# aidilayce/FollowMyHold

Hardware: AMD Instinct MI355X
Metric: guidance-steps/sec (512x512, 778+20k verts) (higher is better)
Workload: dtype f32; 1 GPU; configs[1]: 512x512 frame/GPU, 778-vert hand + 10242-vert/20480-face object, joint step (phase C); images_per_gpu=1, global_images=1, parallelism=image-sharded x1, steps_per_graph=1

## Files before the change

### followmyhold_amd/csrc/foho_step.hip

```cpp
#include <hip/hip_runtime.h>
#include <hip/hip_fp16.h>
#include <stdint.h>
#include <stdlib.h>
#include <string.h>

#include <algorithm>
#include <string>

#include "../../include/foho_hip.h"
#include "foho_common.h"

using namespace foho;

static thread_local char g_err[256] = "";
void foho_set_error(const char* msg) {
    strncpy(g_err, msg, sizeof(g_err) - 1);
    g_err[sizeof(g_err) - 1] = 0;
}
extern "C" const char* foho_last_error(void) { return g_err; }
extern "C" int foho_version(void) { return 105; }
extern "C" int foho_abi_sizes(int64_t out[5]) {
    out[0] = sizeof(foho_image), out[1] = sizeof(foho_dims), out[2] = sizeof(foho_render_cfg), out[3] = sizeof(foho_step_cfg),
    out[4] = sizeof(foho_step_desc);
    return 105;
}

struct ProfState {
    hipEvent_t ev[32];
    const char* name[32];
    int n;
};
static thread_local ProfState* g_prof = nullptr;

#define CHECK_LAUNCH(kname_)                                                                   \
    do {                                                                                     \
        hipError_t e_ = hipGetLastError();                                                   \
        if (e_ != hipSuccess) {                                                              \
            char b_[200];                                                                    \
            snprintf(b_, sizeof(b_), "%s: %s", kname_, hipGetErrorString(e_));                 \
            foho_set_error(b_);                                                              \
            return FOHO_ERR_LAUNCH;                                                          \
        }                                                                                    \
        if (g_prof && g_prof->n < 32) {                                                      \
            g_prof->name[g_prof->n] = kname_;                                                  \
            (void)hipEventRecord(g_prof->ev[g_prof->n++], stream);                           \
        }                                                                                    \
    } while (0)

#include "foho_stamps.h"

constexpr int BTX = 32, BTY = 8;
constexpr int RF = 64;
constexpr int RQ_CAP = 1024;
constexpr int FRAC_SEG = 256;
constexpr int K_SIL = 100;
constexpr int KFIX_MAX = 32;
constexpr int KFIX_FRAGS = 1024;
constexpr int LOSS_BLOCKS = 256;
constexpr int NPART = 12;
constexpr int LOSS_SLOTS = 16;
constexpr int VERT_BLOCKS_MAX = 1024;
constexpr int SIM_NP = 20;
constexpr int VB = 64;
constexpr int VP_CAP = 1024;
constexpr int SIM_ROWS_MAX = VERT_BLOCKS_MAX * (256 / VB);
constexpr int NSTAT = 32;
constexpr int SIM_ACC = 40;
constexpr int STATE_NEXT = 64;
constexpr int PIX_BWD_TILE_BLOCKS = 256;
constexpr int BWD_SPLIT = 4;
constexpr int BWD_SLOTS = 512;

struct MeshInfo {
    unsigned long long kmin_inv[3];
    unsigned long long kmax[3];
};

struct FracEntry {
    int pix;
    int face;
    float sdist;
};
struct KFixEntry {
    int pix;
    int pad;
    unsigned long long thr;
};

constexpr int NSLOT = 64;
struct RSlot {
    unsigned hit_count;
    unsigned rgb_min_inv, rgb_max;
    unsigned disp_min_inv, disp_max;
    unsigned pad[11];
};
struct RStats {
    unsigned flags;
    unsigned pad[3];
};

struct WS {
    size_t total;
    size_t world, ndc, vn_raw, vn, mesh_info, face_ndc;
    size_t p2f, zbuf, sdist, prod, pcol, hit_list, hit_count, bwd_list, bwd_count, tile_touched, tile_clean, pair_v, pending, state_next, sim_acc;
    size_t zkey, fullb, nfrac, plog;
    size_t kfix_count, kfix;
    size_t clean_begin, clean_end;
    size_t frac, frac_count, frac_seg, seg_count, rstats, rslot, loss_part, stats2;
    int nseg;
    size_t g_ndc, g_nrm, g_world, g_direct;
    size_t knn_idx, knn_d2, kp3d, g_kp3d, vert_part, sim_part, xf_part, g_special, parity, int_count, final_ticket, knn_inv, loss_acc, vbox, hand_order;
    size_t tile_static, image_static, act_list, act_count;
    int btiles_x, nbtiles;
    size_t zero_begin, zero_end;
};

static inline size_t al(size_t x) { return (x + 255) & ~(size_t)255; }
static inline int cdiv(int a, int b) { return (a + b - 1) / b; }
static inline int vert_block(const foho_dims& d) { return d.B > 1 ? 2 * VB : VB; }
static inline int raster_faces_per_block(int F, int B = 1) {
    int r = 8;
    while (r < RF && (size_t)r * 256 < (size_t)F * B) r <<= 1;
    return r;
}
constexpr int RF_H_MIN = 2;
static inline void raster_blocks(const foho_dims& d, int& rf_h, int& rf_o, int& nRh, int& nRo, int hand_faces = 0) {
    const int Fh_max = d.Fh_max > 0 ? d.Fh_max : d.Fmax, Fo_max = d.Fo_max > 0 ? d.Fo_max : d.Fmax;
    rf_h = std::max(2, raster_faces_per_block(Fh_max, d.B) / 2);
    if (hand_faces > 0) rf_h = std::max(RF_H_MIN, std::min(hand_faces, RF));
    rf_o = raster_faces_per_block(Fo_max, d.B);
    if (const char* e = FOHO_DEV_ENV("FOHO_DEBUG_RFH")) rf_h = std::max(1, std::min(atoi(e), RF));
    if (const char* e = FOHO_DEV_ENV("FOHO_DEBUG_RFO")) rf_o = std::max(1, std::min(atoi(e), RF));
    nRh = cdiv(Fh_max, rf_h);
    nRo = cdiv(Fo_max, rf_o);
}

static WS make_ws(const foho_dims& d) {
    WS w;
    size_t o = 0;
    const size_t P = (size_t)d.H * d.W, R = d.n_renders, B = d.B;
    const size_t V3 = (size_t)d.Vtot * 3 * 4;
    w.btiles_x = (d.W + BTX - 1) / BTX;
    w.nbtiles = w.btiles_x * ((d.H + BTY - 1) / BTY);
    auto take = [&](size_t bytes) {
        size_t r = o;
        o = al(o + bytes);
        return r;
    };
    const int G1 = d.grid_res + 1;
    w.tile_static = take(B * (size_t)w.nbtiles * 12 * 4);
    w.image_static = take(B * 12 * 8);
    w.zero_begin = o;
    w.frac_count = take(R * B * 4);
    {
        int rf_h, rf_o, nRh, nRo;
#ifdef FOHO_NSEG_AUTO
        raster_blocks(d, rf_h, rf_o, nRh, nRo, 0);
#else
        raster_blocks(d, rf_h, rf_o, nRh, nRo, RF_H_MIN);
#endif
        w.nseg = nRh + nRo;
    }
    w.seg_count = take(R * B * (size_t)w.nseg * 4);
    w.kfix_count = take(R * B * 4);
    w.hit_count = take(R * B * 4);
    w.bwd_count = take(R * B * 4);
    w.rstats = take(R * B * sizeof(RStats));
    w.rslot = take(R * B * NSLOT * sizeof(RSlot));
    w.g_world = take(V3);
    w.g_ndc = take(V3);
    w.g_nrm = take(V3);
    w.parity = take(B * 2 * (size_t)G1 * G1 * 16);
    w.int_count = take(B * 4);
    w.final_ticket = take(B * 4);
    w.loss_acc = take(R * B * LOSS_SLOTS * NPART * 8);
    w.knn_inv = take(B * (size_t)std::max(d.Vh_max, 1) * 8);
    w.zero_end = o;
    w.clean_begin = o;
    w.zkey = take(R * B * P * 8);
    w.fullb = take(R * B * P);
    w.nfrac = take(R * B * P * 4);
    w.plog = take(R * B * P * 8);
    w.tile_touched = take(R * B * (size_t)w.nbtiles);
    w.tile_clean = take(R * B * (size_t)w.nbtiles);
    w.sim_acc = take(2 * B * (size_t)SIM_ACC * 4);
    w.pending = take(B * 4);
    w.clean_end = o;
    w.mesh_info = take(B * 2 * sizeof(MeshInfo));
    w.xf_part = take(B * 2 * VERT_BLOCKS_MAX * 8 * 4);
    w.vbox = take(B * (size_t)VERT_BLOCKS_MAX * 4 * 8 * 4);
    w.world = take(V3);
    w.ndc = take(V3);
    w.vn_raw = take((size_t)d.Vtot * 16);
    w.vn = take(V3);
    w.face_ndc = take((size_t)d.Ftot * 9 * 4);
    w.state_next = take(B * (size_t)STATE_NEXT * 4);
    w.pair_v = take((size_t)d.Ftot * 3 * 8);
    w.p2f = take(R * B * P * 4);
    w.zbuf = take(R * B * P * 4);
    w.sdist = take(R * B * P * 4);
    w.prod = take(R * B * P * 4);
    w.hit_list = take(R * B * (size_t)w.nbtiles * 4);
    w.bwd_list = take(R * B * (size_t)w.nbtiles * BWD_SPLIT * 4);
    w.pcol = take(R * B * P * 12);
    w.frac = take(R * B * (size_t)d.frac_cap * sizeof(FracEntry));
    w.frac_seg = take(R * B * (size_t)w.nseg * FRAC_SEG * sizeof(FracEntry));
    w.act_list = take(R * B * (size_t)w.nbtiles * 4);
    w.act_count = take(R * B * 4);
    w.kfix = take(R * B * KFIX_MAX * sizeof(KFixEntry));
    w.loss_part = take(R * B * LOSS_BLOCKS * NPART * 4);
    w.stats2 = take(R * B * NSTAT * 4);
    w.g_direct = take(V3);
    w.knn_idx = take((size_t)d.Vtot * 4);
    w.knn_d2 = take((size_t)d.Vtot * 4);
    w.hand_order = take(B * (size_t)std::max(d.Vh_max, 1) * 4);
    w.kp3d = take(B * 21 * 3 * 4);
    w.g_kp3d = take(B * 21 * 3 * 4);
    w.vert_part = take(B * VERT_BLOCKS_MAX * 8 * 4);
    w.g_special = take(B * 2 * 6 * 4 * 4);
    w.sim_part = take(B * 2 * (size_t)SIM_ROWS_MAX * SIM_NP * 4);
    w.total = o;
    return w;
}

extern "C" size_t foho_step_workspace_bytes(const foho_dims* dims) {
    if (!dims) return 0;
    return make_ws(*dims).total;
}

extern "C" int64_t foho_step_workspace_region(const foho_dims* dims, int region, int64_t* nbytes) {
    if (!dims) return -1;
    const WS w = make_ws(*dims);
    const foho_dims& d = *dims;
    const size_t P = (size_t)d.H * d.W, R = d.n_renders, B = d.B, V3 = (size_t)d.Vtot * 12;
    const int G1 = d.grid_res + 1;
    size_t off, n;
    switch (region) {
        case FOHO_WS_WORLD: off = w.world; n = V3; break;
        case FOHO_WS_NDC: off = w.ndc; n = V3; break;
        case FOHO_WS_VN: off = w.vn; n = V3; break;
        case FOHO_WS_P2F: off = w.p2f; n = R * B * P * 4; break;
        case FOHO_WS_ZBUF: off = w.zbuf; n = R * B * P * 4; break;
        case FOHO_WS_SDIST: off = w.sdist; n = R * B * P * 4; break;
        case FOHO_WS_PROD: off = w.prod; n = R * B * P * 4; break;
        case FOHO_WS_KNN_IDX: off = w.knn_idx; n = (size_t)d.Vtot * 4; break;
        case FOHO_WS_KNN_D2: off = w.knn_d2; n = (size_t)d.Vtot * 4; break;
        case FOHO_WS_GWORLD: off = w.g_world; n = V3; break;
        case FOHO_WS_FRAC_COUNT: off = w.frac_count; n = R * B * 4; break;
        case FOHO_WS_STATS: off = w.stats2; n = R * B * NSTAT * 4; break;
        case FOHO_WS_PARITY: off = w.parity; n = B * 2 * (size_t)G1 * G1 * 16; break;
        case FOHO_WS_FRAG_COUNT: off = w.nfrac; n = R * B * P * 4; break;
        case FOHO_WS_SEG_COUNT: off = w.seg_count; n = R * B * (size_t)w.nseg * 4; break;
        case FOHO_WS_HAND_ORDER: off = w.hand_order; n = B * (size_t)std::max(d.Vh_max, 1) * 4; break;
        default: return -1;
    }
    if (nbytes) *nbytes = (int64_t)n;
    return (int64_t)off;
}

__device__ __forceinline__ unsigned long long pack_pair(int v0, int v1, int v2, int corner) {
    return (unsigned long long)((unsigned)v0 & 0x3FFFFFu) | ((unsigned long long)((unsigned)(v1 - v0 + (1 << 19)) & 0xFFFFFu) << 22) |
           ((unsigned long long)((unsigned)(v2 - v0 + (1 << 19)) & 0xFFFFFu) << 42) | ((unsigned long long)(corner & 3) << 62);
}
__device__ __forceinline__ void unpack_pair(unsigned long long p, int v[3], int& corner) {
    v[0] = (int)(p & 0x3FFFFFu);
    v[1] = v[0] + (int)((p >> 22) & 0xFFFFFu) - (1 << 19);
    v[2] = v[0] + (int)((p >> 42) & 0xFFFFFu) - (1 << 19);
    corner = (int)(p >> 62);
}

struct Ctx {
    foho_dims d;
    PixAxis ax, ay;
    const foho_image* img;
    const float* verts_in;
    const int32_t* faces;
    const int32_t *inc_off, *inc_fc, *nbr_off, *nbr_idx;
    const float* J;
    const float *tgt_normal, *tgt_disp;
    const uint8_t* mask;
    const float* kps_2d;
    float *params, *adam_m, *adam_v;
    int32_t* adam_t;
    float *losses, *grad_params, *grad_verts_in;
    int32_t* flags;
    float *world, *ndc, *vn_raw, *vn;
    MeshInfo* mesh_info;
    float* face_ndc;
    int32_t* p2f;
    float *zbuf, *sdist, *prod, *pcol;
    int* hit_list;
    unsigned* hit_count;
    int* bwd_list;
    unsigned* bwd_count;
    uint8_t *tile_touched, *tile_clean;
    int* act_list;
    unsigned* act_count;
    unsigned long long* pair_v;
    int* pending;
    float* state_next;
    float* sim_acc;
    unsigned long long* zkey;
    uint8_t* fullb;
    unsigned* nfrac;
    unsigned long long* plog;
    FracEntry* frac;
    unsigned* frac_count;
    FracEntry* frac_seg;
    unsigned* seg_count;
    unsigned* kfix_count;
    KFixEntry* kfix;
    int nseg;
    RStats* rstats;
    RSlot* rslot;
    float *loss_part, *stats2;
    float *g_ndc, *g_nrm, *g_world, *g_direct;
    int32_t* knn_idx;
    const int32_t* hand_order;
    float *knn_d2, *kp3d, *g_kp3d, *vert_part, *sim_part, *xf_part, *g_special, *vbox;
    unsigned long long* parity;
    int32_t* int_count;
    unsigned* final_ticket;
    unsigned long long* knn_inv;
    double* loss_acc;
    float* tile_static;
    double* image_static;
    int btiles_x;
};

__device__ __forceinline__ foho_render_cfg pick_render(const foho_render_cfg (&rr)[2], int r) {
    foho_render_cfg o = rr[0];
    if (r != 0) o = rr[1];
    return o;
}

__device__ __forceinline__ float round_f16(float x) { return __half2float(__float2half(x)); }
__device__ __forceinline__ void gbuf_store(const Ctx& c, size_t pi, float z, const float* col) {
    if (c.d.gbuf_f16) {
        __half* zh = reinterpret_cast<__half*>(c.zbuf);
        __half* ch = reinterpret_cast<__half*>(c.pcol);
        zh[pi] = __float2half(z);
        if (col)
            for (int k = 0; k < 3; k++) ch[3 * pi + k] = __float2half(col[k]);
    } else {
        c.zbuf[pi] = z;
        if (col)
            for (int k = 0; k < 3; k++) c.pcol[3 * pi + k] = col[k];
    }
}
__device__ __forceinline__ void gbuf_load(const Ctx& c, size_t pi, float& z, float* col) {
    if (c.d.gbuf_f16) {
        const __half* zh = reinterpret_cast<const __half*>(c.zbuf);
        const __half* ch = reinterpret_cast<const __half*>(c.pcol);
        z = __half2float(zh[pi]);
        for (int k = 0; k < 3; k++) col[k] = __half2float(ch[3 * pi + k]);
    } else {
        z = c.zbuf[pi];
        for (int k = 0; k < 3; k++) col[k] = c.pcol[3 * pi + k];
    }
}

__device__ __forceinline__ void face_range(const foho_image& im, int face_set, int& f0, int& f1) {
    if (face_set == FOHO_FACES_HAND) {
        f0 = im.f_off;
        f1 = im.f_off + im.Fh;
    } else if (face_set == FOHO_FACES_OBJ) {
        f0 = im.f_off + im.Fh;
        f1 = im.f_off + im.Fh + im.Fo;
    } else {
        f0 = im.f_off;
        f1 = im.f_off + im.Fh + im.Fo;
    }
}

__device__ __forceinline__ void cross3(const float* a, const float* b, float* o) {
    o[0] = a[1] * b[2] - a[2] * b[1];
    o[1] = a[2] * b[0] - a[0] * b[2];
    o[2] = a[0] * b[1] - a[1] * b[0];
}

__device__ __forceinline__ void mesh_center(const MeshInfo& mi, float* cen) {
    for (int k = 0; k < 3; k++) {
        const float mn = ord2f((unsigned)((~mi.kmin_inv[k]) >> 32)), mx = ord2f((unsigned)(mi.kmax[k] >> 32));
        cen[k] = (mn + mx) / 2.0f;
    }
}
__device__ __forceinline__ int mesh_argmin(const MeshInfo& mi, int k) { return (int)(unsigned)((~mi.kmin_inv[k]) & 0xffffffffull); }
__device__ __forceinline__ int mesh_argmax(const MeshInfo& mi, int k) { return (int)(~(unsigned)(mi.kmax[k] & 0xffffffffull)); }

#include "k_vertex.inc"
#include "k_inside.inc"
#include "k_raster.inc"
#include "k_loss.inc"
#include "k_final.inc"
#include "k_xform.inc"
#include "k_backward.inc"
#include "host.inc"
#include "ops.inc"
#include "k_sdf.inc"
#include "k_lbs.inc"
#include "k_icp.inc"
#include "k_flexi.inc"
#include "k_topo.inc"
#include "k_object.inc"
#include "mesh_decimate.inc"
```

### followmyhold_amd/csrc/host.inc

```

static Ctx make_ctx(const foho_step_desc& d, const WS& w) {
    Ctx c;
    memset(&c, 0, sizeof(c));
    char* base = (char*)d.workspace;
    c.d = d.dims;
    c.ax = pix_axis(d.dims.W, d.dims.H);
    c.ay = pix_axis(d.dims.H, d.dims.W);
    c.img = d.images;
    c.verts_in = d.verts_in;
    c.faces = d.faces;
    c.inc_off = d.inc_off;
    c.inc_fc = d.inc_fc;
    c.nbr_off = d.nbr_off;
    c.nbr_idx = d.nbr_idx;
    c.J = d.J_regressor;
    c.tgt_normal = d.tgt_normal;
    c.tgt_disp = d.tgt_disp;
    c.mask = d.mask;
    c.kps_2d = d.kps_2d;
    c.params = d.params;
    c.adam_m = d.adam_m;
    c.adam_v = d.adam_v;
    c.adam_t = d.adam_t;
    c.losses = d.losses;
    c.grad_params = d.grad_params;
    c.grad_verts_in = d.grad_verts_in;
    c.flags = d.flags;
    c.world = (float*)(base + w.world);
    c.ndc = (float*)(base + w.ndc);
    c.vn_raw = (float*)(base + w.vn_raw);
    c.vn = (float*)(base + w.vn);
    c.mesh_info = (MeshInfo*)(base + w.mesh_info);
    c.face_ndc = (float*)(base + w.face_ndc);
    c.p2f = (int32_t*)(base + w.p2f);
    c.zbuf = (float*)(base + w.zbuf);
    c.sdist = (float*)(base + w.sdist);
    c.prod = (float*)(base + w.prod);
    c.pcol = (float*)(base + w.pcol);
    c.hit_list = (int*)(base + w.hit_list);
    c.hit_count = (unsigned*)(base + w.hit_count);
    c.bwd_list = (int*)(base + w.bwd_list);
    c.bwd_count = (unsigned*)(base + w.bwd_count);
    c.tile_touched = (uint8_t*)(base + w.tile_touched);
    c.tile_clean = (uint8_t*)(base + w.tile_clean);
    c.act_list = (int*)(base + w.act_list);
    c.act_count = (unsigned*)(base + w.act_count);
    c.pair_v = (unsigned long long*)(base + w.pair_v);
    c.pending = (int*)(base + w.pending);
    c.state_next = (float*)(base + w.state_next);
    c.sim_acc = (float*)(base + w.sim_acc);
    c.zkey = (unsigned long long*)(base + w.zkey);
    c.fullb = (uint8_t*)(base + w.fullb);
    c.nfrac = (unsigned*)(base + w.nfrac);
    c.plog = (unsigned long long*)(base + w.plog);
    c.frac = (FracEntry*)(base + w.frac);
    c.frac_count = (unsigned*)(base + w.frac_count);
    c.frac_seg = (FracEntry*)(base + w.frac_seg);
    c.seg_count = (unsigned*)(base + w.seg_count);
    c.kfix_count = (unsigned*)(base + w.kfix_count);
    c.kfix = (KFixEntry*)(base + w.kfix);
    c.nseg = w.nseg;
    c.rstats = (RStats*)(base + w.rstats);
    c.rslot = (RSlot*)(base + w.rslot);
    c.loss_part = (float*)(base + w.loss_part);
    c.stats2 = (float*)(base + w.stats2);
    c.g_ndc = (float*)(base + w.g_ndc);
    c.g_nrm = (float*)(base + w.g_nrm);
    c.g_world = (float*)(base + w.g_world);
    c.g_direct = (float*)(base + w.g_direct);
    c.knn_idx = (int32_t*)(base + w.knn_idx);
    c.hand_order = (const int32_t*)(base + w.hand_order);
    c.knn_d2 = (float*)(base + w.knn_d2);
    c.kp3d = (float*)(base + w.kp3d);
    c.g_kp3d = (float*)(base + w.g_kp3d);
    c.vert_part = (float*)(base + w.vert_part);
    c.sim_part = (float*)(base + w.sim_part);
    c.xf_part = (float*)(base + w.xf_part);
    c.vbox = (float*)(base + w.vbox);
    c.g_special = (float*)(base + w.g_special);
    c.parity = (unsigned long long*)(base + w.parity);
    c.int_count = (int32_t*)(base + w.int_count);
    c.final_ticket = (unsigned*)(base + w.final_ticket);
    c.knn_inv = (unsigned long long*)(base + w.knn_inv);
    c.loss_acc = (double*)(base + w.loss_acc);
    c.tile_static = (float*)(base + w.tile_static);
    c.image_static = (double*)(base + w.image_static);
    c.btiles_x = w.btiles_x;
    return c;
}


struct StepPlan {
    int R;
    bool hand_drawn, obj_drawn, knn_on, kps_on, direct_on;
};
static inline StepPlan make_plan(const foho_dims& d, const foho_step_cfg& cfg) {
    StepPlan p;
    p.R = (cfg.n_active_renders > 0 && cfg.n_active_renders < d.n_renders) ? cfg.n_active_renders : d.n_renders;
    p.hand_drawn = p.obj_drawn = false;
    for (int r = 0; r < p.R; r++) {
        p.hand_drawn |= cfg.render[r].face_set != FOHO_FACES_OBJ;
        p.obj_drawn |= cfg.render[r].face_set != FOHO_FACES_HAND;
    }
    const bool lean = cfg.n_active_renders > 0;
    p.knn_on = !lean || cfg.w_contact != 0.0f || cfg.use_intersection;
    p.kps_on = !lean || cfg.w_kps != 0.0f;
    p.direct_on = !lean || cfg.w_edge != 0.0f || cfg.w_verts_obj != 0.0f;
    if (!lean) p.hand_drawn = p.obj_drawn = true;
    return p;
}

static inline bool pair_limits_ok(const foho_dims& d) { return d.Vtot <= (1 << 22) && d.Vmax < (1 << 19) && d.Vh_max + d.Vo_max < (1 << 19); }

__global__ __launch_bounds__(256) void k_zero(uint4* p, size_t n16) {
    const uint4 z = {0u, 0u, 0u, 0u};
    for (size_t i = (size_t)blockIdx.x * 256 + threadIdx.x; i < n16; i += (size_t)gridDim.x * 256) p[i] = z;
}

extern "C" int foho_step_run(const foho_step_desc* desc, const foho_step_cfg* cfg, int stage_mask, void* stream_) {
    if (!desc || !cfg) {
        foho_set_error("foho_step_run: null argument");
        return FOHO_ERR_BAD_ARG;
    }
    const foho_dims& d = desc->dims;
    if (d.B < 1 || d.H < 1 || d.W < 1 || d.H > 8192 || d.W > 8192 || d.n_renders < 1 || d.n_renders > 2 ||
        d.grid_res < 1 || d.grid_res > 127 || d.Vmax < 1 || d.Fmax < 1 || d.frac_cap < 1) {
        foho_set_error("foho_step_run: bad dims");
        return FOHO_ERR_BAD_ARG;
    }
    const WS w = make_ws(d);
    if (!desc->workspace || desc->workspace_bytes < w.total) {
        foho_set_error("foho_step_run: workspace too small (query foho_step_workspace_bytes)");
        return FOHO_ERR_WORKSPACE;
    }
    const int nbv = cdiv(d.Vmax, 256);
    const int nbh = cdiv(d.Vh_max > 0 ? d.Vh_max : 1, 256), nbo = cdiv(d.Vo_max > 0 ? d.Vo_max : 1, 256);
    if (nbv > VERT_BLOCKS_MAX || nbh > VERT_BLOCKS_MAX || nbo > VERT_BLOCKS_MAX) {
        foho_set_error("foho_step_run: more than 262144 vertices per image is not supported");
        return FOHO_ERR_BAD_ARG;
    }
    hipStream_t stream = (hipStream_t)stream_;
    Ctx c = make_ctx(*desc, w);
    const StepPlan plan = make_plan(d, *cfg);
    const int R = plan.R;
    c.d.n_renders = R;
    const int RB = R * d.B;
    if (!pair_limits_ok(d)) {
        foho_set_error("foho_step_run: more than 4194304 vertices per batch or 524287 per image is not supported (pair table)");
        return FOHO_ERR_BAD_ARG;
    }
    if (w.nbtiles > (1 << 16) || d.Fmax >= (1 << 20)) {
        foho_set_error("foho_step_run: image with more than 65536 tiles of 32x8 pixels or mesh with 2^20+ faces is not supported");
        return FOHO_ERR_BAD_ARG;
    }
    if ((stage_mask & (FOHO_STAGE_RASTER | FOHO_STAGE_INSIDE)) && !(stage_mask & FOHO_STAGE_VERTEX)) {
        foho_set_error("foho_step_run: FOHO_STAGE_RASTER / FOHO_STAGE_INSIDE need FOHO_STAGE_VERTEX");
        return FOHO_ERR_BAD_ARG;
    }
    if ((stage_mask & FOHO_STAGE_INSIDE) && !(stage_mask & FOHO_STAGE_RASTER)) {
        foho_set_error("foho_step_run: FOHO_STAGE_INSIDE needs FOHO_STAGE_RASTER");
        return FOHO_ERR_BAD_ARG;
    }
    int sil_bits = 0;
    for (int r = 0; r < R; r++)
        if (cfg->render[r].w_sil != 0.0f) sil_bits |= 1 << r;
    Stage2Cfg s2{};
    s2.nA = nbv;
    s2.knn_chunks = cdiv(std::max(d.Vo_max, 1), KNN_CH);
    s2.hand_order_valid = desc->hand_order_valid ? 1 : 0;
    s2.nC = cdiv(d.Vh_max > 0 ? d.Vh_max : 1, KNN_Q) * s2.knn_chunks;
    raster_blocks(d, s2.rf_h, s2.rf_o, s2.nRh, s2.nRo, desc->hand_faces_per_block);
    const bool do_raster = (stage_mask & FOHO_STAGE_RASTER) != 0;
    if (!do_raster || !plan.hand_drawn) s2.nRh = 0;
    if (!do_raster || !plan.obj_drawn) s2.nRo = 0;
    s2.vn_hand = plan.hand_drawn;
    s2.vn_obj = plan.obj_drawn;
    if (!plan.knn_on) s2.nC = 0;
    s2.if_h = 16;
    s2.lean_h = 256;
    s2.lean_o = s2.lean_i = d.B > 1 ? 64 : 256;
    if (const char* e = FOHO_DEV_ENV("FOHO_DEBUG_LEAN")) {
        int h = 256, o = 64, i = 64;
        if (sscanf(e, "%d,%d,%d", &h, &o, &i) == 3) s2.lean_h = h, s2.lean_o = o, s2.lean_i = i;
    }
    if (const char* e = FOHO_DEV_ENV("FOHO_DEBUG_IFH")) s2.if_h = std::max(1, std::min(atoi(e), 64));
    s2.nIh = cdiv(std::max(d.Fh_max > 0 ? d.Fh_max : d.Fmax, 1), s2.if_h);
    s2.if_o = d.Fo_max >= 4096 ? IFO : IF;
    if (const char* e = FOHO_DEV_ENV("FOHO_DEBUG_IFO")) s2.if_o = atoi(e) == IFO ? IFO : IF;
    s2.nI = ((stage_mask & FOHO_STAGE_INSIDE) && cfg->use_intersection) ? s2.nIh + cdiv(std::max(d.Fo_max > 0 ? d.Fo_max : d.Fmax, 1), s2.if_o) : 0;
    s2.nD = plan.kps_on ? 6 : 0;
    s2.nE = plan.direct_on ? nbo : 0;
    s2.render[0] = cfg->render[0];
    s2.render[1] = cfg->render[1];
    s2.n_renders = R;
    s2.sil_bits = sil_bits;
    s2.dbg = 0;
    s2.blur_radius = cfg->blur_radius;
    s2.sqrt_blur = sqrtf(cfg->blur_radius);
    s2.sigma = cfg->sigma;
#ifdef FOHO_NO_FULLT
    s2.full_t = 0.0f;
#else
    s2.full_t = 20.0f * cfg->sigma;
#endif
    s2.w_edge = cfg->w_edge;
    s2.w_verts = cfg->w_verts_obj;
    s2.w_contact = cfg->w_contact;
    s2.contact_margin = cfg->contact_margin;
    if (const char* dbg = FOHO_DEV_ENV("FOHO_DEBUG_SKIP_ROLES")) {
        const int m = atoi(dbg);
        if (m & 1) s2.nA = 0;
        if (m & 2) s2.nRh = s2.nRo = 0;
        if (m & 32) s2.nI = 0;
        s2.dbg = (m >> 10) & 127;
        if (m & 4) s2.nC = 0;
        if (m & 8) s2.nD = 0;
        if (m & 16) s2.nE = 0;
    }

    BboxCfg bc;
    bc.nbh = nbh;
    bc.nbo = nbo;
    if (stage_mask & FOHO_STAGE_BBOX) {
        hipLaunchKernelGGL(k_bbox_clear, dim3(cdiv(2 * d.B, 64)), dim3(64), 0, stream, c.mesh_info, 2 * d.B);
        CHECK_LAUNCH("k_bbox_clear");
        {
            const size_t n16 = (w.clean_end - w.clean_begin) / 16;
            const int nblk = (int)std::min<size_t>((n16 + 256 * 4 - 1) / (256 * 4), 4096);
            hipLaunchKernelGGL(k_zero, dim3(nblk), dim3(256), 0, stream, (uint4*)((char*)desc->workspace + w.clean_begin), n16);
            CHECK_LAUNCH("k_zero");
        }
        hipLaunchKernelGGL(k_bbox, dim3(nbh + nbo, d.B), dim3(256), 0, stream, c, bc);
        CHECK_LAUNCH("k_bbox");
        hipLaunchKernelGGL(k_pair_table, dim3(cdiv(3 * d.Ftot, 256)), dim3(256), 0, stream, c, 3 * d.Ftot);
        CHECK_LAUNCH("k_pair_table");
    }
    if (stage_mask & FOHO_STAGE_TARGETS) {
        hipLaunchKernelGGL(k_tile_static, dim3(w.nbtiles, d.B), dim3(256), 0, stream, c);
        CHECK_LAUNCH("k_tile_static");
        hipLaunchKernelGGL(k_image_static, dim3(d.B), dim3(256), 0, stream, c, w.nbtiles);
        CHECK_LAUNCH("k_image_static");
    }
    FinalCfg fc{};
    fc.s = *cfg;
    const int vb = vert_block(d);
    const int nvh = cdiv(d.Vh_max > 0 ? d.Vh_max : 1, vb), nvo = cdiv(d.Vo_max > 0 ? d.Vo_max : 1, vb);
    fc.nbh = nvh;
    fc.nbo = nvo;
    fc.nE = s2.nE;
    const bool deferred = cfg->deferred_update && (stage_mask & FOHO_STAGE_STEP) == FOHO_STAGE_STEP;
    fc.deferred = deferred ? 1 : 0;
    const int parity = deferred ? ((cfg->deferred_update - 1) & 1) : 0;
    float* acc_cur = deferred ? c.sim_acc + (size_t)parity * d.B * SIM_ACC : nullptr;
    float* acc_prev = deferred ? c.sim_acc + (size_t)(parity ^ 1) * d.B * SIM_ACC : nullptr;
    fc.acc = acc_prev;
    s2.acc = acc_cur;
    if (stage_mask & FOHO_STAGE_VERTEX) {
        XformCfg xc{};
        xc.deferred = fc.deferred;
        xc.fin = fc;
        xc.nbh = nbh;
        xc.nbo = nbo;
        xc.world_space_input = cfg->world_space_input;
        xc.zero_ptr = (uint4*)((char*)desc->workspace + w.zero_begin);
        xc.zero_n16 = (w.zero_end - w.zero_begin) / 16;
        xc.nz = (int)std::max<size_t>(1, std::min<size_t>(cdiv((int)std::min<size_t>(xc.zero_n16, 1u << 30), 256 * 4 * d.B), 2048));
        hipLaunchKernelGGL(k_xform, dim3(nbh + nbo + xc.nz, d.B), dim3(256), 0, stream, c, xc);
        CHECK_LAUNCH("k_xform");
        hipLaunchKernelGGL(k_stage2, dim3(s2.nC + s2.nRh + s2.nRo + s2.nI + s2.nA + s2.nD + s2.nE, d.B), dim3(256), 0, stream, c, s2);
        CHECK_LAUNCH("k_stage2");
        if (!(stage_mask & FOHO_STAGE_RASTER) && d.Vh_max > 0 && plan.knn_on) {
            hipLaunchKernelGGL(k_knn_decode, dim3(cdiv(d.Vh_max, 256), d.B), dim3(256), 0, stream, c, cfg->w_contact, cfg->contact_margin);
            CHECK_LAUNCH("k_knn_decode");
        }
    }
    if (stage_mask & FOHO_STAGE_RASTER) {
        RasterCfg rc{};
        rc.render[0] = cfg->render[0];
        rc.render[1] = cfg->render[1];
        rc.blur_radius = cfg->blur_radius;
        rc.sqrt_blur = sqrtf(cfg->blur_radius);
        rc.sigma = cfg->sigma;
        rc.gamma = cfg->gamma;
        rc.want_stats = 1;
        rc.sil_bits = sil_bits;
        rc.nbtiles = (int)w.nbtiles;
        rc.coarse_bands = d.B > 1 ? 1 : 0;
        rc.knn_blocks = ((stage_mask & FOHO_STAGE_VERTEX) && d.Vh_max > 0 && plan.knn_on) ? cdiv(d.Vh_max, 256) : 0;
        rc.w_contact = cfg->w_contact;
        rc.contact_margin = cfg->contact_margin;
        if (const char* dbg = FOHO_DEV_ENV("FOHO_DEBUG_SKIP_ROLES"))
            if (atoi(dbg) & 64) rc.want_stats = 2;
        rc.ntile_blocks = rc.nbtiles;
        rc.win_tx0 = rc.win_ty0 = rc.win_w = 0;
        rc.sel_cap = d.B >= 8 ? std::max(64, (int)w.nbtiles * 3 / 8) : 0;
        if (cfg->listed_cap != 0) rc.sel_cap = cfg->listed_cap > 0 ? cfg->listed_cap : 0;
        if (const char* e = FOHO_DEV_ENV("FOHO_DEBUG_RWIN")) {
            int tx0, ty0, ww, wh;
            if (sscanf(e, "%d,%d,%d,%d", &tx0, &ty0, &ww, &wh) == 4 && ww > 0 && wh > 0) {
                rc.win_tx0 = tx0, rc.win_ty0 = ty0, rc.win_w = ww;
                rc.ntile_blocks = ww * wh;
            }
        }
        if (rc.win_w > 0) rc.sel_cap = 0;
        if (rc.sel_cap > 0) {
            rc.ntile_blocks = rc.sel_cap;
            hipLaunchKernelGGL(k_tile_list, dim3(RB), dim3(256), 0, stream, c, rc.nbtiles);
            CHECK_LAUNCH("k_tile_list");
        }
        hipLaunchKernelGGL(k_resolve, dim3(rc.ntile_blocks + rc.knn_blocks, RB), dim3(256), 0, stream, c, rc);
        CHECK_LAUNCH("k_resolve");
        if (rc.sel_cap > 0 && rc.sel_cap < rc.nbtiles) {
            hipLaunchKernelGGL(k_resolve_ovf, dim3(OVF_WG, RB), dim3(256), 0, stream, c, rc);
            CHECK_LAUNCH("k_resolve_ovf");
        }
    }
    if (stage_mask & FOHO_STAGE_LOSS) {
        LossCfg lc{};
        lc.render[0] = cfg->render[0];
        lc.render[1] = cfg->render[1];
        lc.sigma = cfg->sigma;
        lc.gamma = cfg->gamma;
        lc.w_kps = cfg->w_kps;
        lc.use_intersection = cfg->use_intersection;
        lc.kps_on = plan.kps_on;
        lc.nbtiles = w.nbtiles;
        if (const char* e = FOHO_DEV_ENV("FOHO_DEBUG_LOSS")) lc.dbg = atoi(e);
        if (d.B == 1) hipLaunchKernelGGL(k_loss<256>, dim3(256, 2 * d.B), dim3(256), 0, stream, c, lc);
        else if (d.B < 16) hipLaunchKernelGGL(k_loss<128>, dim3(128, 2 * d.B), dim3(256), 0, stream, c, lc);
        else hipLaunchKernelGGL(k_loss<64>, dim3(64, 2 * d.B), dim3(256), 0, stream, c, lc);
        CHECK_LAUNCH("k_loss");
    }
    if (stage_mask & FOHO_STAGE_BACKWARD) {
        BwdCfg bwc{};
        bwc.render[0] = cfg->render[0];
        bwc.render[1] = cfg->render[1];
        bwc.sigma = cfg->sigma;
        bwc.gamma = cfg->gamma;
        bwc.blur_radius = cfg->blur_radius;
        bwc.sqrt_blur = sqrtf(cfg->blur_radius);
        bwc.nbtiles = w.nbtiles;
        bwc.dbg = 0;
        if (const char* dbg = FOHO_DEV_ENV("FOHO_DEBUG_SKIP_ROLES")) bwc.dbg = (atoi(dbg) >> 7) & 7;
        bwc.gtiles = std::min(BWD_SPLIT * w.nbtiles, d.B == 1 ? 2 * PIX_BWD_TILE_BLOCKS : PIX_BWD_TILE_BLOCKS);
        bwc.gfrac = FRAC_BLOCKS;
        if (d.B >= 4) bwc.gtiles = std::min(bwc.gtiles, PIX_BWD_TILE_BLOCKS / 2);
        if (const char* e = FOHO_DEV_ENV("FOHO_DEBUG_GTILES")) bwc.gtiles = std::min(w.nbtiles, atoi(e));
        if (const char* e = FOHO_DEV_ENV("FOHO_DEBUG_GFRAC")) bwc.gfrac = atoi(e);
        hipLaunchKernelGGL(k_pix_bwd, dim3(bwc.gtiles + bwc.gfrac, RB), dim3(256), 0, stream, c, bwc);
        CHECK_LAUNCH("k_pix_bwd");
        VertBwdCfg vc{};
        vc.nbh = nvh;
        vc.nbo = nvo;
        vc.w_contact = cfg->w_contact;
        vc.contact_margin = cfg->contact_margin;
        vc.knn_on = plan.knn_on;
        vc.kps_on = plan.kps_on;
        vc.direct_on = plan.direct_on;
        vc.nrm_hand = plan.hand_drawn;
        vc.nrm_obj = plan.obj_drawn;
        vc.do_final = (stage_mask & FOHO_STAGE_FINAL) ? 1 : 0;
        vc.fin = fc;
        vc.deferred = fc.deferred;
        vc.acc_cur = acc_cur;
        vc.acc_prev = acc_prev;
        if (vb == VB) hipLaunchKernelGGL(k_vert_bwd<VB>, dim3(nvh + nvo, d.B), dim3(256), 0, stream, c, vc);
        else hipLaunchKernelGGL(k_vert_bwd<2 * VB>, dim3(nvh + nvo, d.B), dim3(256), 0, stream, c, vc);
        CHECK_LAUNCH("k_vert_bwd");
    } else if (stage_mask & FOHO_STAGE_FINAL) {
        hipLaunchKernelGGL(k_final, dim3(d.B), dim3(256), 0, stream, c, fc);
        CHECK_LAUNCH("k_final");
    }
    return FOHO_OK;
}

extern "C" int foho_step_finalize(const foho_step_desc* desc, const foho_step_cfg* cfg, void* stream_) {
    if (!desc || !cfg) {
        foho_set_error("foho_step_finalize: null argument");
        return FOHO_ERR_BAD_ARG;
    }
    const foho_dims& d = desc->dims;
    const WS w = make_ws(d);
    if (d.B < 1 || !desc->workspace || desc->workspace_bytes < w.total) {
        foho_set_error("foho_step_finalize: bad dims or workspace too small");
        return FOHO_ERR_WORKSPACE;
    }
    Ctx c = make_ctx(*desc, w);
    const StepPlan plan = make_plan(d, *cfg);
    c.d.n_renders = plan.R;
    FinalCfg fc{};
    fc.s = *cfg;
    fc.nbh = cdiv(d.Vh_max > 0 ? d.Vh_max : 1, vert_block(d));
    fc.nbo = cdiv(d.Vo_max > 0 ? d.Vo_max : 1, vert_block(d));
    fc.nE = plan.direct_on ? cdiv(d.Vo_max > 0 ? d.Vo_max : 1, 256) : 0;
    fc.deferred = 1;
    fc.acc = c.sim_acc + (size_t)((cfg->deferred_update - 1) & 1) * d.B * SIM_ACC;
    hipStream_t stream = (hipStream_t)stream_;
    hipLaunchKernelGGL(k_final, dim3(d.B), dim3(256), 0, stream, c, fc);
    CHECK_LAUNCH("k_final");
    return FOHO_OK;
}

static thread_local const char* g_last_names[FOHO_N_KERNELS];
static thread_local int g_last_n = 0;
extern "C" const char* foho_kernel_name(int i) { return (i >= 0 && i < g_last_n) ? g_last_names[i] : ""; }

extern "C" int foho_step_run_profiled(const foho_step_desc* desc, const foho_step_cfg* cfg, void* stream_, float* ms_out) {
    if (!desc || !cfg || !ms_out) {
        foho_set_error("foho_step_run_profiled: null argument");
        return FOHO_ERR_BAD_ARG;
    }
    hipStream_t stream = (hipStream_t)stream_;
    ProfState ps;
    ps.n = 0;
    hipEvent_t start;
    (void)hipEventCreate(&start);
    for (int i = 0; i < FOHO_N_KERNELS; i++) (void)hipEventCreate(&ps.ev[i]);
    for (int i = 0; i < FOHO_N_KERNELS; i++) ms_out[i] = 0.f;
    {
        foho_step_cfg prev = *cfg;
        if (cfg->deferred_update) prev.deferred_update = (cfg->deferred_update == 1) ? 2 : 1;
        const int rc0 = foho_step_run(desc, &prev, FOHO_STAGE_STEP, stream_);
        if (rc0 != FOHO_OK) return rc0;
    }
    (void)hipEventRecord(start, stream);
    g_prof = &ps;
    const int rc = foho_step_run(desc, cfg, FOHO_STAGE_STEP, stream_);
    g_prof = nullptr;
    (void)hipStreamSynchronize(stream);
    g_last_n = 0;
    if (rc == FOHO_OK) {
        g_last_n = ps.n < FOHO_N_KERNELS ? ps.n : FOHO_N_KERNELS;
        for (int i = 0; i < g_last_n; i++) g_last_names[i] = ps.name[i];
        hipEvent_t prev = start;
        for (int i = 0; i < ps.n && i < FOHO_N_KERNELS; i++) {
            float ms = 0.f;
            (void)hipEventElapsedTime(&ms, prev, ps.ev[i]);
            ms_out[i] = ms;
            prev = ps.ev[i];
        }
    }
    (void)hipEventDestroy(start);
    for (int i = 0; i < FOHO_N_KERNELS; i++) (void)hipEventDestroy(ps.ev[i]);
    return rc;
}
```

### followmyhold_amd/csrc/k_final.inc

```

struct FinalCfg {
    foho_step_cfg s;
    int nbh, nbo, nE;
    float* acc;
    int deferred;
};

struct FinalOut {
    float *params, *m, *v;
    int *t, *flags;
    bool write;
    float* lds_params;
};

__device__ void quat_bwd(const float* q, const float* gR, float* gq) {
    const float r = q[0], i = q[1], j = q[2], k = q[3];
    const float n = ((r * r + i * i) + j * j) + k * k;
    const float ts = 2.0f / n;
    const float A[9] = {-(j * j + k * k), (i * j - k * r), (i * k + j * r), (i * j + k * r), -(i * i + k * k),
                        (j * k - i * r), (i * k - j * r), (j * k + i * r), -(i * i + j * j)};
    float gts = 0.f;
    for (int m = 0; m < 9; m++) gts += gR[m] * A[m];
    const float dr[9] = {0.f, -k, j, k, 0.f, -i, -j, i, 0.f};
    const float di[9] = {0.f, j, k, j, -2.f * i, -r, k, r, -2.f * i};
    const float dj[9] = {-2.f * j, i, r, i, 0.f, k, -r, k, -2.f * j};
    const float dk[9] = {-2.f * k, -r, i, r, -2.f * k, j, i, j, 0.f};
    float g[4] = {0.f, 0.f, 0.f, 0.f};
    for (int m = 0; m < 9; m++) {
        g[0] += gR[m] * dr[m];
        g[1] += gR[m] * di[m];
        g[2] += gR[m] * dj[m];
        g[3] += gR[m] * dk[m];
    }
    const float dts = -ts * ts;
    for (int a = 0; a < 4; a++) gq[a] = ts * g[a] + gts * dts * q[a];
}

__device__ __forceinline__ double pow_int(double x, int n) {
    double r = 1.0;
    while (n > 0) {
        if (n & 1) r *= x;
        x *= x;
        n >>= 1;
    }
    return r;
}

constexpr int FIN_BIAS0 = 128, FIN_LOSS = 96;
struct FinalPre {
    float p, m, v;
    int t_prev;
    float lr;
    int ids[6], my_id;
    float l_kps, lr_[2][3];
    int n_int, fl_prev;
    unsigned rflags;
    float acc_pre;
};
__device__ __forceinline__ void final_prefetch(const Ctx& c, const FinalCfg& cfg, int b, FinalPre& f) {
    const int tid = threadIdx.x;
    f.p = f.m = f.v = 0.f;
    f.acc_pre = 0.f;
    for (int a = 0; a < 6; a++) f.ids[a] = 0;
    f.my_id = 0;
    f.l_kps = 0.f;
    f.n_int = f.fl_prev = 0;
    f.rflags = 0u;
    f.t_prev = 0;
    f.lr = 0.f;
    for (int r = 0; r < 2; r++)
        for (int q = 0; q < 3; q++) f.lr_[r][q] = 0.f;
    if (tid >= FIN_BIAS0 + 16) return;
    const bool bias_lane = tid >= FIN_BIAS0 && tid < FIN_BIAS0 + 16, centre_lane = tid >= 16 && tid < 28;
    if (cfg.deferred && tid < 36) f.acc_pre = cfg.acc[(size_t)b * SIM_ACC + tid];
    if (tid == 0 || bias_lane) f.t_prev = c.adam_t[b];
    if (tid < 16) {
        f.p = c.params[b * 16 + tid];
        f.m = c.adam_m[b * 16 + tid];
        f.v = c.adam_v[b * 16 + tid];
    }
    const int pm = centre_lane ? (tid - 16) / 6 : 0;
    MeshInfo mi;
    if (centre_lane) mi = c.mesh_info[b * 2 + pm];
    if (tid == FIN_LOSS) {
        f.l_kps = c.vert_part[((size_t)b * VERT_BLOCKS_MAX) * 8 + 4];
        f.n_int = 0;
        if (cfg.s.use_intersection)
            f.n_int = cfg.deferred ? __float_as_int(c.stats2[(size_t)b * NSTAT + S_SAFE_INT]) : c.int_count[b];
        f.fl_prev = c.flags[b];
#pragma unroll
        for (int r = 0; r < 2; r++) {
            if (r >= c.d.n_renders) break;
            const float* st = c.stats2 + ((size_t)r * c.d.B + b) * NSTAT;
            f.lr_[r][0] = st[S_L_NORMAL];
            f.lr_[r][1] = st[S_L_DISP];
            f.lr_[r][2] = st[S_L_SIL];
            f.rflags |= cfg.deferred ? (unsigned)__float_as_int(st[S_SAFE_FLAGS]) : c.rstats[(size_t)r * c.d.B + b].flags;
        }
    }
    if (bias_lane) {
        const int lane = tid - FIN_BIAS0;
#pragma unroll
        for (int q = 0; q < 16; q++)
            if (lane == q) f.lr = cfg.s.lr[q];
    }
    if (centre_lane) {
        const foho_image im_ = c.img[b];
        const int nmax = max((pm ? im_.Vo : im_.Vh) - 1, 0);
        for (int a = 0; a < 3; a++) {
            f.ids[2 * a] = min(max(mesh_argmin(mi, a), 0), nmax);
            f.ids[2 * a + 1] = min(max(mesh_argmax(mi, a), 0), nmax);
        }
#pragma unroll
        for (int a = 0; a < 6; a++)
            if ((tid - 16) % 6 == a) f.my_id = f.ids[a];
    }
}

__device__ void final_role(const Ctx& c, const FinalCfg& cfg, int b, const FinalPre& pre, float* red, const FinalOut& out) {
    __shared__ float s_sum[36];
    __shared__ float s_x[5 * 16];
    __shared__ int s_fl;
    const int tid = threadIdx.x;
    const bool dbgf = out.write && b == 0;
    if (dbgf) DBG(90);
    const foho_image im = c.img[b];
    const foho_step_cfg& sc = cfg.s;
    const float p_lane = pre.p, m_lane = pre.m, v_lane = pre.v;
    float v[36];
    for (int q = 0; q < 36; q++) v[q] = 0.f;
    if (cfg.deferred) {
        if (tid < 36) s_sum[tid] = pre.acc_pre;
    } else {
        for (int mesh = 0; mesh < 2; mesh++) {
            const int nb = mesh ? cfg.nbo : cfg.nbh;
            for (int blk = tid; blk < nb; blk += 256) {
                const float* o = c.sim_part + (((size_t)b * 2 + mesh) * SIM_ROWS_MAX + blk) * SIM_NP;
                for (int q = 0; q < 16; q++) v[16 * mesh + q] += o[q];
                if (mesh == 0) {
                    v[32] += o[16];
                    v[33] += o[17];
                }
            }
        }
        for (int blk = tid; blk < cfg.nE; blk += 256) {
            const float* o = c.vert_part + ((size_t)b * VERT_BLOCKS_MAX + blk) * 8;
            v[34] += o[2];
            v[35] += o[3];
        }
    }
    if (tid < 16) s_x[tid] = p_lane;
    float gs3[3] = {0.f, 0.f, 0.f};
    if (tid >= 16 && tid < 28) {
        const float* gs = c.g_special + (((size_t)b * 2 + (tid - 16) / 6) * 6 + (tid - 16) % 6) * 4;
        for (int q = 0; q < 3; q++) gs3[q] = gs[q];
    }
    DBG(15);
    if (cfg.deferred) __syncthreads();
    else block_sum_lds<36>(v, red, s_sum);
    DBG(16);
    if (dbgf) DBG(91);
    const float* s_vp = s_sum + 32;
    const int lane = tid;
    float gq_ = 0.f;
    if (tid < 64) {
        float q4[4];
        {
            const int pl = __float_as_int(p_lane);
            const float qh[4] = {__int_as_float(__builtin_amdgcn_readlane(pl, 4)), __int_as_float(__builtin_amdgcn_readlane(pl, 5)),
                                 __int_as_float(__builtin_amdgcn_readlane(pl, 6)), __int_as_float(__builtin_amdgcn_readlane(pl, 7))};
            const float qo[4] = {__int_as_float(__builtin_amdgcn_readlane(pl, 12)), __int_as_float(__builtin_amdgcn_readlane(pl, 13)),
                                 __int_as_float(__builtin_amdgcn_readlane(pl, 14)), __int_as_float(__builtin_amdgcn_readlane(pl, 15))};
            for (int a = 0; a < 4; a++) q4[a] = ((lane >> 3) & 1) ? qo[a] : qh[a];
        }
        if (lane < 16) {
            const int mesh = lane >> 3, j = lane & 7;
            const float* sm = s_sum + 16 * mesh;
            if (j == 0) {
                gq_ = sm[3];
            } else if (j < 4) {
                const float wt = mesh ? sc.w_trans_obj : sc.w_trans_hand;
                gq_ = sm[j - 1] + wt * 2.0f * p_lane / 3.0f;
            } else {
                float g4[4];
                quat_bwd(q4, sm + 4, g4);
                gq_ = g4[j - 4];
            }
            if (out.write) c.grad_params[b * 16 + lane] = gq_;
        } else if (lane < 28) {
            const int mesh = (lane - 16) / 6;
            if ((mesh ? im.Vo : im.Vh) > 0) {
                float gm[3] = {gs3[0], gs3[1], gs3[2]};
#pragma unroll
                for (int a = 0; a < 6; a++)
                    if (pre.ids[a] == pre.my_id) gm[a >> 1] += 0.5f * s_sum[16 * mesh + 13 + (a >> 1)];
                const int vtx = im.v_off + (mesh ? im.Vh : 0) + pre.my_id;
                if (!out.write) {
                } else if (mesh) {
                    const float* M = im.T_h2m;
                    c.grad_verts_in[3 * vtx] = (gm[0] * M[0] + gm[1] * M[4]) + gm[2] * M[8];
                    c.grad_verts_in[3 * vtx + 1] = (gm[0] * M[1] + gm[1] * M[5]) + gm[2] * M[9];
                    c.grad_verts_in[3 * vtx + 2] = (gm[0] * M[2] + gm[1] * M[6]) + gm[2] * M[10];
                } else {
                    for (int q = 0; q < 3; q++) c.grad_verts_in[3 * vtx + q] = gm[q];
                }
            }
        }
        if (dbgf) DBG(92);
    } else if (tid == FIN_LOSS) {
        const float th0 = s_x[1], th1 = s_x[2], th2 = s_x[3];
        const float to0 = s_x[9], to1 = s_x[10], to2 = s_x[11];
        float* L = c.losses + (size_t)b * FOHO_N_LOSS;
        const float l_kps = pre.l_kps;
        const int n_int = pre.n_int, fl_prev = pre.fl_prev;
        const unsigned rflags = pre.rflags;
        float lr_[2][3];
        for (int r = 0; r < 2; r++)
            for (int q = 0; q < 3; q++) lr_[r][q] = pre.lr_[r][q];
        const float Vh = (float)im.Vh;
        const float l_contact = (im.Vo > 0) ? s_vp[0] / Vh : 0.f;
        const float mean_d2 = (im.Vo > 0) ? s_vp[1] / Vh : 0.f;
        const float l_edge = (im.n_edges > 0) ? s_vp[2] / (float)im.n_edges : 0.f;
        const float l_verts = (im.Vo > 0) ? s_vp[3] / (3.0f * (float)im.Vo) : 0.f;
        const float l_th = ((th0 * th0 + th1 * th1) + th2 * th2) / 3.0f, l_to = ((to0 * to0 + to1 * to1) + to2 * to2) / 3.0f;
        float w_int = 0.f, l_int = 0.f;
        if (sc.use_intersection) {
            l_int = (float)n_int / 1000.0f;
            w_int = (mean_d2 < sc.int_gate && sc.int_gate_step_ok) ? sc.w_int_near : sc.w_int_far;
        }
        float total = w_int * l_int;
        total += sc.w_contact * l_contact;
#pragma unroll
        for (int r = 0; r < 2; r++) {
            if (r >= c.d.n_renders) break;
            const foho_render_cfg rc = pick_render(sc.render, r);
            if (rc.w_normal != 0.f) total += rc.w_normal * lr_[r][0];
            if (rc.w_disp != 0.f) total += rc.w_disp * lr_[r][1];
            if (rc.w_sil != 0.f) total += rc.w_sil * lr_[r][2];
        }
        if (sc.w_verts_obj != 0.f) total += sc.w_verts_obj * l_verts;
        if (sc.w_edge != 0.f) total += sc.w_edge * l_edge;
        if (sc.w_trans_obj != 0.f) total += sc.w_trans_obj * l_to;
        if (sc.w_kps != 0.f) total += sc.w_kps * l_kps;
        if (sc.w_trans_hand != 0.f) total += sc.w_trans_hand * l_th;
        if (out.write) {
            L[FOHO_L_TOTAL] = total;
            L[FOHO_L_INTERSECTION] = l_int;
            L[FOHO_L_CONTACT] = l_contact;
            L[FOHO_L_KPS] = l_kps;
            L[FOHO_L_TRANS_HAND] = l_th;
            L[FOHO_L_TRANS_OBJ] = l_to;
            L[FOHO_L_VERTS_OBJ] = l_verts;
            L[FOHO_L_EDGE] = l_edge;
            L[FOHO_L_NORMAL0] = lr_[0][0];
            L[FOHO_L_DISP0] = lr_[0][1];
            L[FOHO_L_SIL0] = lr_[0][2];
            L[FOHO_L_NORMAL1] = lr_[1][0];
            L[FOHO_L_DISP1] = lr_[1][1];
            L[FOHO_L_SIL1] = lr_[1][2];
            L[FOHO_L_N_INTERSECT] = (float)n_int;
            L[FOHO_L_W_INT] = w_int;
            L[FOHO_L_MEAN_D2] = mean_d2;
        }
        int fl = fl_prev | (int)(rflags & 14u);
        if (total != total) fl |= 1;
        if (out.write) out.flags[0] = fl;
        s_fl = fl;
    } else if (tid >= FIN_BIAS0 && tid < FIN_BIAS0 + 16) {
        const int l = tid - FIN_BIAS0;
        const int t = pre.t_prev + 1;
        const double bc1 = 1.0 - pow_int((double)sc.beta1, t), bc2 = 1.0 - pow_int((double)sc.beta2, t);
        s_x[16 + l] = (float)sqrt(bc2);
        s_x[32 + l] = (float)((double)pre.lr / bc1);
        s_x[48 + l] = (float)(1.0 - (double)pre.lr * (double)sc.weight_decay);
        s_x[64 + l] = pre.lr;
    }
    __syncthreads();
    if (dbgf) DBG(93);
    if (tid < 16) {
        const int fl = s_fl;
        const float bc2s = s_x[16 + lane], step_size = s_x[32 + lane], decay = s_x[48 + lane], lr = s_x[64 + lane];
        const bool update = sc.do_update && !(fl & (1 | 16 | 32 | 64));
        float pv = p_lane, m = m_lane, vv = v_lane;
        if (update && lr != 0.f) {
            if (sc.weight_decay != 0.f) pv = pv * decay;
            m = m + (gq_ - m) * (1.0f - sc.beta1);
            vv = vv * sc.beta2 + (1.0f - sc.beta2) * gq_ * gq_;
            const float denom = sqrtf(vv) / bc2s + sc.eps;
            pv = pv - step_size * (m / denom);
        }
        if (out.lds_params) out.lds_params[lane] = pv;
        if (out.write && ((update && lr != 0.f) || out.lds_params)) {
            out.params[lane] = pv;
            out.m[lane] = m;
            out.v[lane] = vv;
        }
        if (lane == 0 && out.write && (update || out.lds_params)) out.t[0] = update ? pre.t_prev + 1 : pre.t_prev;
    }
    if (dbgf) DBG(94);
}

__device__ __forceinline__ FinalOut final_out_in_place(const Ctx& c, int b) {
    return FinalOut{c.params + b * 16, c.adam_m + b * 16, c.adam_v + b * 16, c.adam_t + b, c.flags + b, true, nullptr};
}

__global__ __launch_bounds__(256) void k_final(Ctx c, FinalCfg cfg) {
    __shared__ float red[36 * 16];
    const int b = blockIdx.x;
    if (cfg.deferred && !c.pending[b]) return;
    FinalPre pre;
    final_prefetch(c, cfg, b, pre);
    final_role(c, cfg, b, pre, red, final_out_in_place(c, b));
    if (cfg.deferred) {
        __syncthreads();
        if (threadIdx.x < SIM_ACC) cfg.acc[(size_t)b * SIM_ACC + threadIdx.x] = 0.f;
        if (threadIdx.x == 0) c.pending[b] = 0;
    }
}
```

### followmyhold_amd/csrc/k_inside.inc

```

struct DirEdge {
    float ax, ay, bx, by;
    float sgn;
    bool tie;
};
__device__ __forceinline__ DirEdge make_edge(int i, int j, float xi, float yi, float xj, float yj) {
    DirEdge e;
    if (i < j) {
        e.ax = xi; e.ay = yi; e.bx = xj; e.by = yj; e.sgn = 1.0f;
    } else {
        e.ax = xj; e.ay = yj; e.bx = xi; e.by = yi; e.sgn = -1.0f;
    }
    const float dx = xj - xi, dy = yj - yi;
    e.tie = (dy < 0.0f) || (dy == 0.0f && dx > 0.0f);
    return e;
}
__device__ __forceinline__ bool left_of(const DirEdge& d, float px, float py, float& e_out) {
    float e = (d.bx - d.ax) * (py - d.ay) - (d.by - d.ay) * (px - d.ax);
    if (d.sgn < 0.0f) e = -e;
    e_out = e;
    if (e > 0.0f) return true;
    if (e < 0.0f) return false;
    return d.tie;
}

__device__ __forceinline__ void tab_range(const float* tab, int G1, float lo, float hi, int& i0, int& i1) {
    int a = 0, b = G1;
    while (a < b) {
        const int m = (a + b) >> 1;
        if (tab[m] < lo) a = m + 1;
        else b = m;
    }
    i0 = a;
    a = 0;
    b = G1;
    while (a < b) {
        const int m = (a + b) >> 1;
        if (tab[m] <= hi) a = m + 1;
        else b = m;
    }
    i1 = a - 1;
}

__device__ __forceinline__ void inside_candidate(const Ctx& c, const float* V, int ia, int ib, int ic, int ix, int iy, const float* tab,
                                                 int G1, int b, int mesh) {
    const DirEdge e_bc = make_edge(ib, ic, V[3], V[4], V[6], V[7]);
    const DirEdge e_ca = make_edge(ic, ia, V[6], V[7], V[0], V[1]);
    const DirEdge e_ab = make_edge(ia, ib, V[0], V[1], V[3], V[4]);
    const float px = tab[ix], py = tab[G1 + iy];
    float e0, e1, e2;
    const bool s0 = left_of(e_bc, px, py, e0);
    const bool s1 = left_of(e_ca, px, py, e1);
    const bool s2 = left_of(e_ab, px, py, e2);
    if (!((s0 && s1 && s2) || (!s0 && !s1 && !s2))) return;
    const float area = (e0 + e1) + e2;
    if (area == 0.0f) return;
    const float zh = ((e0 * V[2] + e1 * V[5]) + e2 * V[8]) / area;
    int a = 0, bnd = G1;
    while (a < bnd) {
        const int m = (a + bnd) >> 1;
        if (tab[2 * G1 + m] < zh) a = m + 1;
        else bnd = m;
    }
    const int kz = a;
    if (kz <= 0) return;
    const unsigned long long mlo = (kz >= 64) ? ~0ull : ((1ull << kz) - 1ull);
    const unsigned long long mhi = (kz > 64) ? ((kz - 64 >= 64) ? ~0ull : ((1ull << (kz - 64)) - 1ull)) : 0ull;
    unsigned long long* w = c.parity + (((size_t)b * 2 + mesh) * G1 * G1 + (size_t)ix * G1 + iy) * 2;
    atomicXor(&w[0], mlo);
    if (mhi) atomicXor(&w[1], mhi);
}

constexpr int IF = 64;
constexpr int IFO = 256;
struct InsideLds {
    float tab[3 * 128];
    float box[12];
    float vx[IF * 9];
    int vid[IF * 3];
    short4 cbox[IF];
    unsigned off[IF + 1];
};

__device__ void inside_faces_role(const Ctx& c, const Stage2Cfg& cfg, int b, int blk, InsideLds& L) {
    const foho_image im = c.img[b];
    const int res = c.d.grid_res, G1 = res + 1;
    const int tid = threadIdx.x;
    const bool hand_blk = blk < cfg.nIh;
    const bool direct = !hand_blk && cfg.if_o == IFO;
    const int nper = hand_blk ? cfg.if_h : (direct ? IFO : IF);
    const int lf0 = hand_blk ? blk * cfg.if_h : im.Fh + (blk - cfg.nIh) * nper;
    const int lf_end = hand_blk ? im.Fh : im.Fh + im.Fo;
    const int lean = direct ? 256 : cfg.lean_i;
    if (lf0 >= lf_end || tid >= lean) return;
    const int lf = lf0 + tid;
    const bool live = tid < nper && lf < lf_end;
    int id[3] = {0, 0, 0};
    float P[9] = {0.f, 0.f, 0.f, 0.f, 0.f, 0.f, 0.f, 0.f, 0.f};
    if (live) {
        const int f = im.f_off + lf;
        for (int k = 0; k < 3; k++) id[k] = c.faces[3 * f + k];
        for (int k = 0; k < 3; k++)
            for (int q = 0; q < 3; q++) P[3 * k + q] = c.world[3 * id[k] + q];
    }
    world_boxes(c, im, b, L.box);
    fill_grid_table(c, L.box, L.tab, lean);
    __syncthreads();
    if (direct) {
        if (!live) return;
        const float wx0 = fmaxf(L.box[0], L.box[6]), wx1 = fminf(L.box[3], L.box[9]);
        const float wy0 = fmaxf(L.box[1], L.box[7]), wy1 = fminf(L.box[4], L.box[10]);
        const float xlo = fmaxf(fminf(fminf(P[0], P[3]), P[6]), wx0), xhi = fminf(fmaxf(fmaxf(P[0], P[3]), P[6]), wx1);
        const float ylo = fmaxf(fminf(fminf(P[1], P[4]), P[7]), wy0), yhi = fminf(fmaxf(fmaxf(P[1], P[4]), P[7]), wy1);
        if (!(xlo <= xhi && ylo <= yhi)) return;
        int ix0, ix1, iy0, iy1;
        tab_range(L.tab, G1, xlo, xhi, ix0, ix1);
        tab_range(L.tab + G1, G1, ylo, yhi, iy0, iy1);
        for (int ix = ix0; ix <= ix1; ix++)
            for (int iy = iy0; iy <= iy1; iy++) inside_candidate(c, P, id[0], id[1], id[2], ix, iy, L.tab, G1, b, 1);
        return;
    }
    if (tid < IF) {
        int ix0 = 1, ix1 = 0, iy0 = 1, iy1 = 0;
        if (live) {
            const float wx0 = fmaxf(L.box[0], L.box[6]), wx1 = fminf(L.box[3], L.box[9]);
            const float wy0 = fmaxf(L.box[1], L.box[7]), wy1 = fminf(L.box[4], L.box[10]);
            const float xmin = fminf(fminf(P[0], P[3]), P[6]), xmax = fmaxf(fmaxf(P[0], P[3]), P[6]);
            const float ymin = fminf(fminf(P[1], P[4]), P[7]), ymax = fmaxf(fmaxf(P[1], P[4]), P[7]);
            tab_range(L.tab, G1, fmaxf(xmin, wx0), fminf(xmax, wx1), ix0, ix1);
            tab_range(L.tab + G1, G1, fmaxf(ymin, wy0), fminf(ymax, wy1), iy0, iy1);
        }
        const bool valid = live && ix0 <= ix1 && iy0 <= iy1;
        short4 cb;
        cb.x = (short)ix0;
        cb.y = (short)ix1;
        cb.z = (short)iy0;
        cb.w = (short)iy1;
        L.cbox[tid] = cb;
        for (int k = 0; k < 9; k++) L.vx[tid * 9 + k] = P[k];
        for (int k = 0; k < 3; k++) L.vid[tid * 3 + k] = id[k];
        const unsigned area = valid ? (unsigned)(ix1 - ix0 + 1) * (unsigned)(iy1 - iy0 + 1) : 0u;
        const unsigned incl = wave_incl_scan(area);
        L.off[tid] = incl - area;
        if (tid == IF - 1) L.off[IF] = incl;
    }
    __syncthreads();
    const unsigned T = FOHO_ABLATED(cfg, 32) ? 0u : L.off[IF];
    for (unsigned t = tid; t < T; t += lean) {
        int s = 0;
#pragma unroll
        for (int step = IF / 2; step > 0; step >>= 1)
            if (L.off[s + step] <= t) s += step;
        const short4 cb = L.cbox[s];
        const unsigned o = t - L.off[s];
        const unsigned ny = (unsigned)(cb.w - cb.z + 1);
        unsigned qx = (unsigned)((float)o * __builtin_amdgcn_rcpf((float)ny));
        int ry = (int)o - (int)(qx * ny);
        if (ry < 0) {
            qx--;
            ry += (int)ny;
        } else if (ry >= (int)ny) {
            qx++;
            ry -= (int)ny;
        }
        const int ix = cb.x + (int)qx, iy = cb.z + ry;
        inside_candidate(c, &L.vx[s * 9], L.vid[s * 3], L.vid[s * 3 + 1], L.vid[s * 3 + 2], ix, iy, L.tab, G1, b, hand_blk ? 0 : 1);
    }
}
```

### followmyhold_amd/csrc/k_raster.inc

```

struct Shade {
    float rgb[3], col[3], p, wnum, delta, den;
};

__device__ __forceinline__ void shade_from_col(const foho_image& im, const float* col, float z, float sd, float sigma, float gamma,
                                               Shade& s) {
    s.p = sigmoidf(-sd / sigma);
    const float z_inv = (im.zfar - z) / (im.zfar - im.znear);
    const float z_inv_max = fmaxf(z_inv, 1e-10f);
    s.wnum = s.p * expf((z_inv - z_inv_max) / gamma);
    s.delta = fmaxf(expf((1e-10f - z_inv_max) / gamma), 1e-10f);
    s.den = s.wnum + s.delta;
    for (int k = 0; k < 3; k++) {
        s.col[k] = col[k];
        s.rgb[k] = (s.wnum * s.col[k] + s.delta * 1.0f) / s.den;
    }
}
__device__ __forceinline__ void face_colour(const Ctx& c, size_t gf, float* col) {
    const int i0 = c.faces[3 * gf], i1 = c.faces[3 * gf + 1], i2 = c.faces[3 * gf + 2];
    for (int k = 0; k < 3; k++) col[k] = (c.vn[3 * i0 + k] + c.vn[3 * i1 + k]) + c.vn[3 * i2 + k];
}

struct RasterCfg {
    foho_render_cfg render[2];
    float blur_radius, sqrt_blur, sigma, gamma;
    int want_stats;
    int sil_bits;
    int coarse_bands;
    int nbtiles;
    int ntile_blocks;
    int win_tx0, win_ty0, win_w;
    int sel_cap;
    int knn_blocks;
    float w_contact, contact_margin;
};


constexpr double LOG_FIX = 1099511627776.0;
__device__ __forceinline__ unsigned long long neg_log2_fixed(float om) {
    return (unsigned long long)(long long)__double2ll_rn(-log2((double)om) * LOG_FIX);
}
__device__ __forceinline__ float prod_from_fixed(unsigned long long s) {
    return (float)exp2(-(double)s * (1.0 / LOG_FIX));
}


struct RasterLds {
    float fv[RF * 9];
    float ec[RF * 9];
    short4 box[RF];
    unsigned off[RF + 1];
    unsigned q[RQ_CAP];
    unsigned nq;
    unsigned nfr[2];
    unsigned long long clipmask;
};

__device__ __forceinline__ bool render_has_face(int face_set, bool is_hand) {
    return !((face_set == FOHO_FACES_HAND && !is_hand) || (face_set == FOHO_FACES_OBJ && is_hand));
}

__device__ void role_raster(const Ctx& c, const foho_image& im, const Stage2Cfg& cfg, int b, int blk, RasterLds& rl) {
    const int tid = threadIdx.x;
    const int H = c.d.H, W = c.d.W;
    const bool objblk = blk >= cfg.nRh;
    const int fpb = objblk ? cfg.rf_o : cfg.rf_h;
    const int lb = objblk ? blk - cfg.nRh : blk;
    const int nFm = objblk ? im.Fo : im.Fh;
    const int lean = objblk ? cfg.lean_o : cfg.lean_h;
    if (lb * fpb >= nFm || tid >= lean) return;
    FOHO_ABLATE_RETURN(cfg, 64);
    const int lf0 = (objblk ? im.Fh : 0) + lb * fpb;
    if (tid == 0) {
        rl.nq = 0;
        rl.nfr[0] = rl.nfr[1] = 0;
    }
    const bool dbgr = b == 0 && (blk == cfg.nRh / 2 || blk == cfg.nRh + cfg.nRo / 2);
    const int dslot = (blk < cfg.nRh) ? 50 : 60;
    (void)dslot;
    if (dbgr) DBG(dslot);
    unsigned rmask = 0u;
    for (int r = 0; r < 2; r++)
        if (r < cfg.n_renders && render_has_face(pick_render(cfg.render, r).face_set, !objblk)) rmask |= 1u << r;
    if (tid < RF) {
        const int lf = lf0 + tid;
        bool valid = false, clipped = false;
        int x0 = 1, x1 = 0, y0 = 1, y1 = 0;
        float fv[9] = {0.f, 0.f, 0.f, 0.f, 0.f, 0.f, 0.f, 0.f, 0.f};
        if (tid < fpb && lb * fpb + tid < nFm) {
            const int f = im.f_off + lf;
            int vi[3];
            for (int k = 0; k < 3; k++) vi[k] = c.faces[3 * f + k];
            if (dbgr) DBGW(dslot + 6);
            for (int k = 0; k < 3; k++) {
                fv[3 * k] = c.ndc[3 * vi[k]];
                fv[3 * k + 1] = c.ndc[3 * vi[k] + 1];
                fv[3 * k + 2] = c.ndc[3 * vi[k] + 2];
            }
            if (dbgr) DBGW(dslot + 7);
            for (int k = 0; k < 9; k++) {
                FOHO_UNLESS_ABLATED(cfg, 8) c.face_ndc[9 * (size_t)f + k] = fv[k];
                rl.fv[tid * 9 + k] = fv[k];
            }
            if (dbgr) DBG(dslot + 30);
            const bool member = rmask != 0u;
            const float zmax = fmaxf(fmaxf(fv[2], fv[5]), fv[8]);
            const float zmin = fminf(fminf(fv[2], fv[5]), fv[8]);
            const float farea = edge_fn(fv[0], fv[1], fv[3], fv[4], fv[6], fv[7]);
            const float zclip = im.znear * 0.5f;
            const bool near_cull = zmax < zclip;
            clipped = member && !near_cull && zmin < zclip;
            valid = member && !near_cull && !(zmax < 0.0f) && (clipped || !(farea <= K_EPS && farea >= -K_EPS));
            if (valid) {
                float xlo = fminf(fminf(fv[0], fv[3]), fv[6]) - cfg.sqrt_blur;
                float xhi = fmaxf(fmaxf(fv[0], fv[3]), fv[6]) + cfg.sqrt_blur;
                float ylo = fminf(fminf(fv[1], fv[4]), fv[7]) - cfg.sqrt_blur;
                float yhi = fmaxf(fmaxf(fv[1], fv[4]), fv[7]) + cfg.sqrt_blur;
                if (__builtin_expect(clipped, 0)) {
                    float t0[9], t1[9];
                    const ClipGeom g = clip_subtris(fv, zclip, t0, t1);
                    xlo = fminf(fminf(t0[0], t0[3]), t0[6]);
                    xhi = fmaxf(fmaxf(t0[0], t0[3]), t0[6]);
                    ylo = fminf(fminf(t0[1], t0[4]), t0[7]);
                    yhi = fmaxf(fmaxf(t0[1], t0[4]), t0[7]);
                    if (g.n == 2) {
                        xlo = fminf(xlo, fminf(fminf(t1[0], t1[3]), t1[6]));
                        xhi = fmaxf(xhi, fmaxf(fmaxf(t1[0], t1[3]), t1[6]));
                        ylo = fminf(ylo, fminf(fminf(t1[1], t1[4]), t1[7]));
                        yhi = fmaxf(yhi, fmaxf(fmaxf(t1[1], t1[4]), t1[7]));
                    }
                    xlo -= cfg.sqrt_blur;
                    xhi += cfg.sqrt_blur;
                    ylo -= cfg.sqrt_blur;
                    yhi += cfg.sqrt_blur;
                }
                valid = (xlo == xlo) && (xhi == xhi) && (ylo == ylo) && (yhi == yhi);
                if (dbgr) DBG(dslot + 31);
                if (valid) {
                    ndc_to_pix_range(xlo, xhi, c.ax, x0, x1);
                    ndc_to_pix_range(ylo, yhi, c.ay, y0, y1);
                    valid = (x0 <= x1) && (y0 <= y1);
                }
                if (dbgr) DBG(dslot + 32);
                if (valid && !FOHO_ABLATED(cfg, 4)) {
                    const int tx0 = x0 / BTX, tx1 = x1 / BTX, ty0 = y0 / BTY, ty1 = y1 / BTY;
                    const size_t tplane = (size_t)c.btiles_x * ((H + BTY - 1) / BTY);
                    for (int r = 0; r < 2; r++) {
                        if (!((rmask >> r) & 1u)) continue;
                        uint8_t* tt = c.tile_touched + ((size_t)r * c.d.B + b) * tplane;
                        if (tx1 - tx0 <= 1 && ty1 - ty0 <= 1) {
                            tt[ty0 * c.btiles_x + tx0] = 1;
                            tt[ty0 * c.btiles_x + tx1] = 1;
                            tt[ty1 * c.btiles_x + tx0] = 1;
                            tt[ty1 * c.btiles_x + tx1] = 1;
                        } else {
                            for (int ty = ty0; ty <= ty1; ty++)
                                for (int tx = tx0; tx <= tx1; tx++) tt[ty * c.btiles_x + tx] = 1;
                        }
                    }
                }
            }
        }
        if (dbgr) DBG(dslot + 9);
        {
            float ec[9] = {0.f, 0.f, 1.f, 0.f, 0.f, 1.f, 0.f, 0.f, 1.f};
            if (valid && !clipped) {
                const float x0 = fv[0], y0 = fv[1], x1 = fv[3], y1 = fv[4], x2 = fv[6], y2 = fv[7];
                const float area = edge_fn(x2, y2, x0, y0, x1, y1) + K_EPS;
                if (fabsf(area) > 1e-7f && fv[2] > 0.f && fv[5] > 0.f && fv[8] > 0.f) {
                    const float sgn = (area > 0.f) ? 1.0f : -1.0f;
                    const float reject_d = cfg.sqrt_blur * 1.01f + 1e-5f;
                    const float ex[3] = {x2 - x1, x0 - x2, x1 - x0}, ey[3] = {y2 - y1, y0 - y2, y1 - y0};
                    const float bx_[3] = {x1, x2, x0}, by_[3] = {y1, y2, y0};
#pragma unroll
                    for (int k = 0; k < 3; k++) {
                        const float A = sgn * ey[k], Bc = -sgn * ex[k];
                        const float C = sgn * __builtin_fmaf(by_[k], ex[k], -(bx_[k] * ey[k]));
                        const float aA = fabsf(A), aB = fabsf(Bc);
                        const float len1 = aA + aB;
                        const float bound = 4e-6f * __builtin_fmaf(aA, c.ax.offset + fabsf(bx_[k]), aB * (c.ay.offset + fabsf(by_[k])));
                        ec[3 * k] = A;
                        ec[3 * k + 1] = Bc;
                        ec[3 * k + 2] = C + __builtin_fmaf(reject_d, len1, bound);
                    }
                }
            }
            for (int k = 0; k < 9; k++) rl.ec[tid * 9 + k] = ec[k];
        }
        short4 box;
        box.x = (short)(valid ? x0 : 1);
        box.y = (short)(valid ? x1 : 0);
        box.z = (short)(valid ? y0 : 1);
        box.w = (short)(valid ? y1 : 0);
        rl.box[tid] = box;
        const unsigned long long cm = __ballot(valid && clipped);
        if (tid == 0) rl.clipmask = cm;
        const unsigned area = valid ? (unsigned)(x1 - x0 + 1) * (unsigned)(y1 - y0 + 1) : 0u;
        const unsigned incl = wave_incl_scan(area);
        rl.off[tid] = incl - area;
        if (tid == RF - 1) rl.off[RF] = incl;
    }
    if (dbgr) DBG(dslot + 1);
    __syncthreads();
    if (dbgr) DBG(dslot + 2);
    const unsigned T = FOHO_ABLATED(cfg, 32) ? 0u : rl.off[RF];
    const size_t P = (size_t)H * W;

    for (unsigned t0 = 0; t0 < T; t0 += RQ_CAP) {
        const unsigned tend = min(T, t0 + (unsigned)RQ_CAP);
        for (unsigned t = t0 + tid; t < tend; t += lean) {
            int s = 0;
#pragma unroll
            for (int step = RF / 2; step > 0; step >>= 1)
                if (rl.off[s + step] <= t) s += step;
            const short4 bx = rl.box[s];
            const unsigned o = t - rl.off[s];
            const unsigned bw = (unsigned)(bx.y - bx.x + 1);
            unsigned row = (unsigned)((float)o * __builtin_amdgcn_rcpf((float)bw));
            int col = (int)o - (int)(row * bw);
            if (col < 0) {
                row--;
                col += (int)bw;
            } else if (col >= (int)bw) {
                row++;
                col -= (int)bw;
            }
            const int px = bx.x + col, py = bx.z + (int)row;
            {
                const float xf = pix_to_ndc(W - 1 - px, c.ax), yf = pix_to_ndc(H - 1 - py, c.ay);
                const float* ec = &rl.ec[s * 9];
                const float e0 = __builtin_fmaf(ec[0], xf, __builtin_fmaf(ec[1], yf, ec[2]));
                const float e1 = __builtin_fmaf(ec[3], xf, __builtin_fmaf(ec[4], yf, ec[5]));
                const float e2 = __builtin_fmaf(ec[6], xf, __builtin_fmaf(ec[7], yf, ec[8]));
                if (fminf(fminf(e0, e1), e2) < 0.f) continue;
            }
            const unsigned q = atomicAdd(&rl.nq, 1u);
            rl.q[q] = ((unsigned)s << 26) | ((unsigned)py << 13) | (unsigned)px;
        }
        if (dbgr) DBG(dslot + 3);
        __syncthreads();
        if (dbgr) DBG(dslot + 4);
        const unsigned nq = FOHO_ABLATED(cfg, 16) ? 0u : rl.nq;
        for (unsigned q = tid; q < nq; q += lean) {
            const unsigned item = rl.q[q];
            const int s = item >> 26, py = (item >> 13) & 8191, px = item & 8191;
            float fv[9];
            for (int k = 0; k < 9; k++) fv[k] = rl.fv[s * 9 + k];
            Frag fr;
            {
                const float xf = pix_to_ndc(W - 1 - px, c.ax), yf = pix_to_ndc(H - 1 - py, c.ay);
                bool ok;
                if (__builtin_expect((rl.clipmask >> s) & 1ull, 0)) {
                    int sub;
                    ok = eval_frag_near(fv, im.znear * 0.5f, xf, yf, cfg.blur_radius, cfg.sqrt_blur, fr, sub);
                } else {
                    ok = eval_frag<true>(fv, xf, yf, cfg.blur_radius, cfg.sqrt_blur, fr, cfg.full_t);
                }
                if (!ok) continue;
            }
            const int lf = lf0 + s;
            const bool is_hand = !objblk;
            const int pix = py * W + px;
            const unsigned zb = __float_as_uint(fr.z);
            for (int r = 0; r < cfg.n_renders; r++) {
                const int fs = pick_render(cfg.render, r).face_set;
                if (!render_has_face(fs, is_hand)) continue;
                const unsigned frel = (unsigned)((fs == FOHO_FACES_OBJ) ? lf - im.Fh : lf);
                const size_t rb = (size_t)r * c.d.B + b;
                const unsigned long long key = ((unsigned long long)zb << 32) | frel;
                FOHO_UNLESS_ABLATED(cfg, 2) atomicMax(&c.zkey[rb * P + pix], ~key);
                if ((cfg.sil_bits >> r) & 1) {
                    const float om = (fr.sdist == -INFINITY) ? 0.0f : 1.0f - sigmoidf(-fr.sdist / cfg.sigma);
                    if (om == 0.0f) {
                        FOHO_UNLESS_ABLATED(cfg, 1) c.fullb[rb * P + pix] = 1;
                    } else {
                        atomicAdd(&c.nfrac[rb * P + pix], 1u);
                        atomicAdd(&c.plog[rb * P + pix], neg_log2_fixed(om));
                        const unsigned li = (r == 0) ? atomicAdd(&rl.nfr[0], 1u) : atomicAdd(&rl.nfr[1], 1u);
                        if (li < (unsigned)FRAC_SEG) {
                            c.frac_seg[(rb * c.nseg + blk) * (size_t)FRAC_SEG + li] = FracEntry{pix, (int)frel, fr.sdist};
                        } else {
                            const unsigned slot = atomicAdd(&c.frac_count[rb], 1u);
                            if (slot < (unsigned)c.d.frac_cap) c.frac[rb * (size_t)c.d.frac_cap + slot] = FracEntry{pix, (int)frel, fr.sdist};
                            else atomicOr(&c.rstats[rb].flags, 2u);
                        }
                    }
                }
            }
        }
        if (dbgr) DBG(dslot + 5);
        if (tend < T) {
            __syncthreads();
            if (tid == 0) rl.nq = 0;
            __syncthreads();
        }
    }
    __syncthreads();
    if (tid < 2 && rl.nfr[tid] > 0) c.seg_count[((size_t)tid * c.d.B + b) * c.nseg + blk] = min(rl.nfr[tid], (unsigned)FRAC_SEG);
    if (dbgr && tid == 0) DBG_VALUE(dslot + 8, T);
}

__global__ __launch_bounds__(256) __attribute__((amdgpu_waves_per_eu(7, 7))) void k_stage2(Ctx c, Stage2Cfg cfg) {
    KSPAN(1);
    __shared__ float red[32];
    constexpr size_t knn_lds = (size_t)KNN_ST * 12 + 256 * 8;
    constexpr size_t ri_lds = sizeof(RasterLds) > sizeof(InsideLds) ? sizeof(RasterLds) : sizeof(InsideLds);
    __shared__ __align__(16) unsigned char s_raw[ri_lds > knn_lds ? ri_lds : knn_lds];
    RasterLds& rl = *reinterpret_cast<RasterLds*>(s_raw);
    {
        int k = (int)blockIdx.x - cfg.nC, lean_role = 256;
        if (k >= 0) {
            if (k < cfg.nRh) lean_role = cfg.lean_h;
            else if (k < cfg.nRh + cfg.nRo) lean_role = cfg.lean_o;
            else if (k - cfg.nRh - cfg.nRo < cfg.nI) lean_role = (k - cfg.nRh - cfg.nRo < cfg.nIh || cfg.if_o != IFO) ? cfg.lean_i : 256;
        }
        if ((int)threadIdx.x >= lean_role) return;
    }
    const int b = blockIdx.y;
    const foho_image im = c.img[b];
    int blk = blockIdx.x;
    if (blk < cfg.nC) return role_knn(c, im, cfg, b, xcd_order(blk, cfg.nC), s_raw);
    blk -= cfg.nC;
    if (blk < cfg.nRh + cfg.nRo)
        return role_raster(c, im, cfg, b, blk < cfg.nRh ? blk : cfg.nRh + xcd_order(blk - cfg.nRh, cfg.nRo), rl);
    blk -= cfg.nRh + cfg.nRo;
    if (blk < cfg.nI)
        return inside_faces_role(c, cfg, b, blk < cfg.nIh ? blk : cfg.nIh + xcd_order(blk - cfg.nIh, cfg.nI - cfg.nIh),
                                 *reinterpret_cast<InsideLds*>(s_raw));
    blk -= cfg.nI;
    if (blk < cfg.nA) return role_normals(c, im, cfg, xcd_order(blk, cfg.nA));
    blk -= cfg.nA;
    if (blk < cfg.nD) return role_kps(c, im, b, blk);
    blk -= cfg.nD;
    if (blk < cfg.nE) return role_obj_local(c, im, cfg, b, xcd_order(blk, cfg.nE), red);
}

__device__ __forceinline__ void kbuffer_fix(const Ctx& c, const RasterCfg& cfg, const foho_image& im, int rbi, int f0r, int f1r, int px,
                                         int py, bool need_fix) {
    __shared__ unsigned long long s_key[KFIX_FRAGS];
    __shared__ unsigned s_n, s_full;
    __shared__ unsigned long long s_log;
    __shared__ int s_px, s_py;
    const int tid = threadIdx.x, H = c.d.H, W = c.d.W;
    const float zclip = im.znear * 0.5f;
    for (int owner = 0; owner < 256; owner++) {
        __syncthreads();
        if (tid == owner) {
            s_px = need_fix ? px : -1;
            s_py = py;
            s_n = 0;
            s_full = 0;
            s_log = 0ull;
        }
        __syncthreads();
        const int qx = s_px, qy = s_py;
        if (qx < 0) continue;
        const float xf = pix_to_ndc(W - 1 - qx, c.ax), yf = pix_to_ndc(H - 1 - qy, c.ay);
        for (int s = tid; s < KFIX_FRAGS; s += 256) s_key[s] = ~0ull;
        __syncthreads();
        for (int f = f0r + tid; f < f1r; f += 256) {
            float fv[9];
            for (int k = 0; k < 9; k++) fv[k] = c.face_ndc[9 * (size_t)f + k];
            Frag fr;
            int sub;
            if (!eval_frag_near(fv, zclip, xf, yf, cfg.blur_radius, cfg.sqrt_blur, fr, sub)) continue;
            const unsigned slot = atomicAdd(&s_n, 1u);
            if (slot < (unsigned)KFIX_FRAGS) s_key[slot] = ((unsigned long long)__float_as_uint(fr.z) << 32) | (unsigned)(f - f0r);
        }
        __syncthreads();
        const unsigned n = s_n;
        const size_t pi = (size_t)rbi * H * W + (size_t)qy * W + qx;
        if (n > (unsigned)KFIX_FRAGS) {
            if (tid == 0) atomicOr(&c.rstats[rbi].flags, 4u);
            continue;
        }
        for (unsigned k = 2; k <= (unsigned)KFIX_FRAGS; k <<= 1)
            for (unsigned j = k >> 1; j > 0; j >>= 1) {
                for (unsigned t = tid; t < (unsigned)KFIX_FRAGS; t += 256) {
                    const unsigned u = t ^ j;
                    if (u > t) {
                        const unsigned long long a = s_key[t], b = s_key[u];
                        const bool up = (t & k) == 0;
                        if ((a > b) == up) {
                            s_key[t] = b;
                            s_key[u] = a;
                        }
                    }
                }
                __syncthreads();
            }
        const unsigned kept = min(n, (unsigned)K_SIL);
        if (tid < (int)kept) {
            const int f = f0r + (int)(unsigned)(s_key[tid] & 0xffffffffull);
            float fv[9];
            for (int k = 0; k < 9; k++) fv[k] = c.face_ndc[9 * (size_t)f + k];
            Frag fr;
            int sub;
            eval_frag_near(fv, zclip, xf, yf, cfg.blur_radius, cfg.sqrt_blur, fr, sub);
            const float om = 1.0f - sigmoidf(-fr.sdist / cfg.sigma);
            if (om == 0.0f) atomicOr(&s_full, 1u);
            else atomicAdd(&s_log, neg_log2_fixed(om));
        }
        __syncthreads();
        if (tid == 0) {
            c.prod[pi] = s_full ? 0.0f : prod_from_fixed(s_log);
            const unsigned slot = atomicAdd(&c.kfix_count[rbi], 1u);
            if (slot < (unsigned)KFIX_MAX) c.kfix[(size_t)rbi * KFIX_MAX + slot] = KFixEntry{qy * W + qx, 0, s_key[kept - 1]};
            else atomicOr(&c.rstats[rbi].flags, 4u);
        }
    }
    __syncthreads();
}

__global__ __launch_bounds__(256) void k_tile_list(Ctx c, int nbtiles) {
    __shared__ unsigned s_wtot[4];
    __shared__ unsigned s_base;
    const size_t rb = blockIdx.x;
    const uint8_t* tt = c.tile_touched + rb * nbtiles;
    const uint8_t* tc = c.tile_clean + rb * nbtiles;
    int* out = c.act_list + rb * nbtiles;
    if (threadIdx.x == 0) s_base = 0u;
    __syncthreads();
    for (int t0 = 0; t0 < nbtiles; t0 += 1024) {
        const int t = t0 + 4 * (int)threadIdx.x;
        unsigned act = 0u;
        for (int j = 0; j < 4; j++)
            if (t + j < nbtiles && (tt[t + j] || !tc[t + j])) act |= 1u << j;
        const unsigned cnt = (unsigned)__popc(act);
        const unsigned incl = wave_incl_scan(cnt);
        if (lane_id() == 63) s_wtot[wave_id()] = incl;
        __syncthreads();
        unsigned off = s_base + incl - cnt;
        for (int w = 0; w < wave_id(); w++) off += s_wtot[w];
        for (int j = 0; j < 4; j++)
            if ((act >> j) & 1u) out[off++] = t + j;
        __syncthreads();
        if (threadIdx.x == 0) s_base += s_wtot[0] + s_wtot[1] + s_wtot[2] + s_wtot[3];
        __syncthreads();
    }
    if (threadIdx.x == 0) c.act_count[rb] = s_base;
}

constexpr int OVF_WG = 128;
__device__ __forceinline__ void resolve_one(const Ctx& c, const RasterCfg& cfg, int rbi, int tile, float* s_red, unsigned* s_hits, unsigned* s_fixw) {
    const int r = rbi / c.d.B, b = rbi % c.d.B;
    const size_t rb = rbi;
    const int H = c.d.H, W = c.d.W, P = H * W;
    const int tx = tile % c.btiles_x, ty = tile / c.btiles_x;
    const int px = tx * BTX + (threadIdx.x % BTX), py = ty * BTY + (threadIdx.x / BTX);
    const bool in_img = px < W && py < H;
    const int i = py * W + px;
    const bool dbgt = rbi == c.d.B && tile == c.btiles_x * (c.d.H / BTY / 2) + c.btiles_x / 2;
    if (dbgt) DBG(70);
    if (dbgt) DBG(71);
    const foho_image im = c.img[b];
    int f0r, f1r;
    face_range(im, pick_render(cfg.render, r).face_set, f0r, f1r);
    const bool sil = (cfg.sil_bits >> r) & 1;
    float mn = INFINITY, mx = -INFINITY, dmn = INFINITY, dmx = -INFINITY;
    unsigned hit = 0;
    int fwin = -1;
    bool need_fix = false;
    if (in_img) {
        const size_t pi = rb * (size_t)P + i;
        const unsigned long long inv = c.zkey[pi];
        if (dbgt) DBG(72);
        if (inv != 0ull) c.zkey[pi] = 0ull;
        if (inv == 0ull) {
            c.p2f[pi] = -1;
        } else {
            const unsigned long long key = ~inv;
            const int f = (int)(unsigned)(key & 0xffffffffull);
            const float z = __uint_as_float((unsigned)(key >> 32));
            const size_t gf = (size_t)(f + f0r);
            float fv[9];
            for (int k = 0; k < 9; k++) fv[k] = c.face_ndc[9 * gf + k];
            Frag fr;
            if (dbgt) DBG(73);
            {
                const float xf = pix_to_ndc(W - 1 - px, c.ax), yf = pix_to_ndc(H - 1 - py, c.ay), zclip = im.znear * 0.5f;
                if (__builtin_expect(fminf(fminf(fv[2], fv[5]), fv[8]) < zclip, 0)) {
                    int sub;
                    eval_frag_near(fv, zclip, xf, yf, cfg.blur_radius, cfg.sqrt_blur, fr, sub);
                } else {
                    fr.sdist = winner_sdist(fv, xf, yf);
                }
            }
            if (dbgt) DBG(74);
            float prod = 0.0f;
            if (sil) {
                const uint8_t full = c.fullb[pi];
                const unsigned long long pl = c.plog[pi];
                if (full) c.fullb[pi] = 0;
                if (pl != 0ull) {
                    c.plog[pi] = 0ull;
                    const unsigned nfr = c.nfrac[pi];
                    c.nfrac[pi] = 0u;
                    need_fix = nfr >= (unsigned)K_SIL && (nfr > (unsigned)K_SIL || full);
                    if (!full) prod = prod_from_fixed(pl);
                }
            }
            fwin = f;
            c.p2f[pi] = f;
            c.sdist[pi] = fr.sdist;
            c.prod[pi] = prod;
            float zs = z;
            if (c.d.gbuf_f16) zs = round_f16(z);
            if (!cfg.want_stats) gbuf_store(c, pi, zs, nullptr);
            if (cfg.want_stats) {
                Shade sh;
                float col[3];
                if (dbgt) DBG(75);
                face_colour(c, gf, col);
                if (dbgt) DBG(76);
                if (c.d.gbuf_f16)
                    for (int k = 0; k < 3; k++) col[k] = round_f16(col[k]);
                gbuf_store(c, pi, zs, col);
                shade_from_col(im, col, zs, fr.sdist, cfg.sigma, cfg.gamma, sh);
                for (int k = 0; k < 3; k++) {
                    mn = fminf(mn, sh.rgb[k]);
                    mx = fmaxf(mx, sh.rgb[k]);
                }
                const float disp = 1.0f / (zs + 1e-6f);
                dmn = disp;
                dmx = disp;
                hit = 1;
            }
        }
    }
    if (dbgt) DBG(77);
    const unsigned long long hb = __ballot(hit != 0);
    const int fleft = __shfl_up(fwin, 1);
    const unsigned long long headb = __ballot(fwin >= 0 && ((threadIdx.x % BTX) == 0 || fleft != fwin));
    const unsigned long long fixb = __ballot(need_fix);
    if (lane_id() == 0) s_fixw[wave_id()] = fixb != 0ull ? 1u : 0u;
    const int any_hit = __syncthreads_or(hit != 0);
    if (__builtin_expect((s_fixw[0] | s_fixw[1] | s_fixw[2] | s_fixw[3]) != 0u, 0)) kbuffer_fix(c, cfg, im, rbi, f0r, f1r, px, py, need_fix);
    if (dbgt) DBG(78);
    unsigned hslot = 0u;
    if (threadIdx.x == 0) {
        if (any_hit) hslot = atomicAdd(&c.hit_count[rb], 1u);
        c.tile_touched[rb * cfg.nbtiles + tile] = 0;
        c.tile_clean[rb * cfg.nbtiles + tile] = (uint8_t)(any_hit ? 0 : 1);
    }
    if (any_hit) {
        mn = wave_min(mn);
        mx = wave_max(mx);
        dmn = wave_min(dmn);
        dmx = wave_max(dmx);
        const int wv = wave_id();
        if (lane_id() == 0) {
            s_red[wv] = mn;
            s_red[4 + wv] = mx;
            s_red[8 + wv] = dmn;
            s_red[12 + wv] = dmx;
            s_hits[wv] = (unsigned)__popcll(hb) | ((unsigned)__popcll(headb) << 16);
        }
        __syncthreads();
        if (threadIdx.x == 0) {
            const unsigned nhh = s_hits[0] + s_hits[1] + s_hits[2] + s_hits[3];
            const unsigned nh = nhh & 0xffffu, nruns = nhh >> 16;
            const unsigned parts = cfg.coarse_bands ? ((nh > 160u && 3u * nruns > 480u) ? 2u : 1u) : ((nh > 160u) ? 4u : ((nh > 80u) ? 2u : 1u));
            const unsigned base = atomicAdd(&c.bwd_count[rb], parts);
            c.hit_list[(size_t)rb * cfg.nbtiles + hslot] = tile;
            for (unsigned p = 0; p < parts; p++) c.bwd_list[(size_t)rb * cfg.nbtiles * BWD_SPLIT + base + p] = (int)((unsigned)tile | (p << 16) | (parts << 20));
            if (cfg.want_stats != 2) {
                RSlot* st = &c.rslot[rb * NSLOT + (tile % NSLOT)];
                atomicAdd(&st->hit_count, nh);
                const unsigned k0 = ~f2ord(fminf(fminf(s_red[0], s_red[1]), fminf(s_red[2], s_red[3])));
                const unsigned k1 = f2ord(fmaxf(fmaxf(s_red[4], s_red[5]), fmaxf(s_red[6], s_red[7])));
                const unsigned k2 = ~f2ord(fminf(fminf(s_red[8], s_red[9]), fminf(s_red[10], s_red[11])));
                const unsigned k3 = f2ord(fmaxf(fmaxf(s_red[12], s_red[13]), fmaxf(s_red[14], s_red[15])));
                atomicMax(&st->rgb_min_inv, k0);
                atomicMax(&st->rgb_max, k1);
                atomicMax(&st->disp_min_inv, k2);
                atomicMax(&st->disp_max, k3);
            }
        }
    }
    if (dbgt) DBG(79);
}

__global__ __launch_bounds__(256) __attribute__((amdgpu_waves_per_eu(8, 8))) void k_resolve(Ctx c, RasterCfg cfg) {
    KSPAN(2);
    __shared__ float s_red[4 * 4];
    __shared__ unsigned s_hits[4];
    __shared__ unsigned s_fixw[4];
    const int rbi = blockIdx.y;
    if ((int)blockIdx.x >= cfg.ntile_blocks) {
        if (rbi < c.d.B) knn_decode(c, c.img[rbi], cfg.w_contact, cfg.contact_margin, rbi, (int)blockIdx.x - cfg.ntile_blocks);
        return;
    }
    int tile = blockIdx.x;
    if (cfg.sel_cap > 0) {
        const int entry = c.act_list[(size_t)rbi * cfg.nbtiles + min((int)blockIdx.x, cfg.nbtiles - 1)];
        if (blockIdx.x >= c.act_count[rbi]) return;
        tile = entry;
    } else {
        if (FOHO_ABLATED_WINDOW && cfg.win_w > 0) tile = (cfg.win_ty0 + (int)blockIdx.x / cfg.win_w) * c.btiles_x + cfg.win_tx0 + (int)blockIdx.x % cfg.win_w;
        const size_t ti = (size_t)rbi * cfg.nbtiles + tile;
        if (!c.tile_touched[ti] && c.tile_clean[ti]) return;
    }
    resolve_one(c, cfg, rbi, tile, s_red, s_hits, s_fixw);
}

__global__ __launch_bounds__(256) void k_resolve_ovf(Ctx c, RasterCfg cfg) {
    __shared__ float s_red[4 * 4];
    __shared__ unsigned s_hits[4];
    __shared__ unsigned s_fixw[4];
    const int rbi = blockIdx.y;
    const unsigned n = c.act_count[rbi];
#pragma clang loop unroll(disable)
    for (unsigned rank = (unsigned)cfg.sel_cap + blockIdx.x; rank < n; rank += OVF_WG) {
        resolve_one(c, cfg, rbi, c.act_list[(size_t)rbi * cfg.nbtiles + rank], s_red, s_hits, s_fixw);
        __syncthreads();
    }
}
```

### followmyhold_amd/csrc/k_vertex.inc

```

__device__ __forceinline__ void load_moge(const Ctx& c, const foho_image& im, int mesh, int gi, float* v) {
    const float x = c.verts_in[3 * gi], y = c.verts_in[3 * gi + 1], z = c.verts_in[3 * gi + 2];
    if (mesh == 0) {
        v[0] = x;
        v[1] = y;
        v[2] = z;
    } else {
        const float* M = im.T_h2m;
        v[0] = ((x * M[0] + y * M[1]) + z * M[2]) + M[3];
        v[1] = ((x * M[4] + y * M[5]) + z * M[6]) + M[7];
        v[2] = ((x * M[8] + y * M[9]) + z * M[10]) + M[11];
    }
}

struct BboxCfg {
    int nbh, nbo;
};
__global__ __launch_bounds__(64) void k_bbox_clear(MeshInfo* mi, int n) {
    const int i = blockIdx.x * 64 + threadIdx.x;
    if (i < n)
        for (int a = 0; a < 3; a++) mi[i].kmin_inv[a] = mi[i].kmax[a] = 0ull;
}
__device__ void bbox_role(const Ctx& c, const BboxCfg& cfg, int bx, int b) {
    __shared__ unsigned long long s_k[6][4];
    const foho_image im = c.img[b];
    const int mesh = (bx < cfg.nbh) ? 0 : 1;
    const int blk = mesh ? (bx - cfg.nbh) : bx;
    const int n = mesh ? im.Vo : im.Vh;
    if (blk * 256 >= n) return;
    const int base = im.v_off + (mesh ? im.Vh : 0);
    const int i = blk * 256 + threadIdx.x;
    unsigned long long k[6] = {0ull, 0ull, 0ull, 0ull, 0ull, 0ull};
    if (i < n) {
        float v[3];
        load_moge(c, im, mesh, base + i, v);
        for (int a = 0; a < 3; a++) {
            const unsigned long long o = (unsigned long long)f2ord(v[a]) << 32;
            k[a] = ~(o | (unsigned)i);
            k[3 + a] = o | (unsigned)(~(unsigned)i);
        }
    }
    for (int a = 0; a < 6; a++) {
        unsigned long long x = k[a];
#pragma unroll
        for (int o = 32; o > 0; o >>= 1) {
            const unsigned long long y = __shfl_down(x, o, 64);
            x = (y > x) ? y : x;
        }
        if (lane_id() == 0) s_k[a][wave_id()] = x;
    }
    __syncthreads();
    if (threadIdx.x < 6) {
        unsigned long long x = s_k[threadIdx.x][0];
        for (int w = 1; w < 4; w++) x = (s_k[threadIdx.x][w] > x) ? s_k[threadIdx.x][w] : x;
        MeshInfo* mi = &c.mesh_info[b * 2 + mesh];
        unsigned long long* dst = (threadIdx.x < 3) ? &mi->kmin_inv[threadIdx.x] : &mi->kmax[threadIdx.x - 3];
        atomicMax(dst, x);
    }
}
__global__ __launch_bounds__(256) void k_bbox(Ctx c, BboxCfg cfg) { bbox_role(c, cfg, (int)blockIdx.x, (int)blockIdx.y); }

__global__ __launch_bounds__(256) void k_pair_table(Ctx c, int n) {
    const int e = blockIdx.x * 256 + threadIdx.x;
    if (e >= n) return;
    const int fc = c.inc_fc[e], f = fc >> 2;
    c.pair_v[e] = pack_pair(c.faces[3 * f], c.faces[3 * f + 1], c.faces[3 * f + 2], fc & 3);
}

__device__ void world_boxes(const Ctx& c, const foho_image& im, int b, float* s_box) {
    if (wave_id() == 0) {
        float v[12];
        for (int mesh = 0; mesh < 2; mesh++) {
            for (int a = 0; a < 3; a++) {
                v[6 * mesh + a] = INFINITY;
                v[6 * mesh + 3 + a] = -INFINITY;
            }
            const int nb = ((mesh ? im.Vo : im.Vh) + 255) / 256;
            for (int blk = lane_id(); blk < nb; blk += 64) {
                const float* row = c.xf_part + (((size_t)b * 2 + mesh) * VERT_BLOCKS_MAX + blk) * 8;
                for (int a = 0; a < 3; a++) {
                    v[6 * mesh + a] = fminf(v[6 * mesh + a], row[a]);
                    v[6 * mesh + 3 + a] = fmaxf(v[6 * mesh + 3 + a], row[3 + a]);
                }
            }
        }
        for (int q = 0; q < 12; q++) {
            const float x = ((q % 6) < 3) ? wave_min(v[q]) : wave_max(v[q]);
            if (lane_id() == 0) s_box[q] = x;
        }
    }
    __syncthreads();
}

struct Stage2Cfg {
    int nA, nC, nD, nE, nI;
    int lean_h, lean_o, lean_i;
    int nIh, if_h, if_o;
    float* acc;
    int knn_chunks;
    int hand_order_valid;
    int nRh, nRo, rf_h, rf_o;
    foho_render_cfg render[2];
    int n_renders, sil_bits;
    bool vn_hand, vn_obj;
    int dbg;
    float blur_radius, sqrt_blur, sigma;
    float full_t;
    float w_edge, w_verts, w_contact, contact_margin;
};

__device__ void role_normals(const Ctx& c, const foho_image& im, const Stage2Cfg& cfg, int blk) {
    const int i = blk * 256 + threadIdx.x;
    if (i >= im.Vh + im.Vo) return;
    if (!((i < im.Vh) ? cfg.vn_hand : cfg.vn_obj)) return;
    const int gv = im.v_off + i;
    float acc[3] = {0.f, 0.f, 0.f};
    const int e0 = c.inc_off[gv], e1 = c.inc_off[gv + 1];
    for (int base = e0; base < e1; base += 8) {
        int fid[8], vi[8][3];
        float P[8][9];
#pragma unroll
        for (int u = 0; u < 8; u++) fid[u] = c.inc_fc[min(base + u, e1 - 1)] >> 2;
#pragma unroll
        for (int u = 0; u < 8; u++)
            for (int k = 0; k < 3; k++) vi[u][k] = c.faces[3 * fid[u] + k];
#pragma unroll
        for (int u = 0; u < 8; u++)
            for (int k = 0; k < 3; k++)
                for (int q = 0; q < 3; q++) P[u][3 * k + q] = c.world[3 * vi[u][k] + q];
#pragma unroll
        for (int u = 0; u < 8; u++) {
            if (base + u >= e1) break;
            float A[3], Bv[3], n[3];
            for (int k = 0; k < 3; k++) {
                A[k] = P[u][6 + k] - P[u][3 + k];
                Bv[k] = P[u][k] - P[u][3 + k];
            }
            cross3(A, Bv, n);
            acc[0] += n[0];
            acc[1] += n[1];
            acc[2] += n[2];
        }
    }
    const float nrm = sqrtf((acc[0] * acc[0] + acc[1] * acc[1]) + acc[2] * acc[2]);
    const float den = fmaxf(nrm, 1e-6f);
    for (int k = 0; k < 3; k++) c.vn[3 * gv + k] = acc[k] / den;
    const float inv = 1.0f / den;
    const bool reg = nrm > 1e-6f;
    reinterpret_cast<float4*>(c.vn_raw)[gv] = make_float4(reg ? acc[0] * inv : 0.0f, reg ? acc[1] * inv : 0.0f, reg ? acc[2] * inv : 0.0f, inv);
}

template <bool P2>
__device__ __forceinline__ void ndc_to_pix_range_t(float lo, float hi, const PixAxis& ax, int& p0, int& p1) {
    const int S1 = ax.S1;
    const float off = ax.offset;
    auto centre = [&](int i) {
        const float num = ax.range * (float)i + ax.offset;
        return -ax.offset + (P2 ? num * ax.inv_s1 : num / ax.s1);
    };
    const float nlo = (lo + off) * ax.s1 - off, nhi = (hi + off) * ax.s1 - off;
    float flo = P2 ? nlo * ax.inv_range : nlo / ax.range;
    float fhi = P2 ? nhi * ax.inv_range : nhi / ax.range;
    flo = fminf(fmaxf(flo, -2.0f), ax.s1 + 1.0f);
    fhi = fminf(fmaxf(fhi, -2.0f), ax.s1 + 1.0f);
    int i0 = max(0, (int)ceilf(flo)), i1 = min(S1 - 1, (int)floorf(fhi));
    const int e0 = min(i0, S1), e1 = max(i1, -1);
    bool a[4], b[4];
#pragma unroll
    for (int k = 0; k < 4; k++) {
        const int ia = e0 - 2 + k, ib = e1 - 1 + k;
        a[k] = (ia >= S1) | ((ia >= 0) & (centre(ia) >= lo));
        b[k] = (ib < 0) | ((ib < S1) & (centre(ib) <= hi));
    }
    if (a[0] | !a[3] | !b[0] | b[3]) {
        i0 = 0;
        while (i0 < S1 && centre(i0) < lo) i0++;
        i1 = S1 - 1;
        while (i1 >= 0 && centre(i1) > hi) i1--;
    } else {
        i0 = a[1] ? e0 - 1 : (a[2] ? e0 : e0 + 1);
        i1 = b[2] ? e1 + 1 : (b[1] ? e1 : e1 - 1);
    }
    p0 = S1 - 1 - i1;
    p1 = S1 - 1 - i0;
}
__device__ __forceinline__ void ndc_to_pix_range(float lo, float hi, const PixAxis& ax, int& p0, int& p1) {
    if (ax.pow2 && ax.range_pow2) ndc_to_pix_range_t<true>(lo, hi, ax, p0, p1);
    else ndc_to_pix_range_t<false>(lo, hi, ax, p0, p1);
}
__device__ __forceinline__ void ndc_to_pix_range(float lo, float hi, int S1, int S2, int& p0, int& p1) {
    ndc_to_pix_range(lo, hi, pix_axis(S1, S2), p0, p1);
}

constexpr int KNN_Q = 64, KNN_CH = 1024, KNN_GRP = 8;
constexpr int KNN_ST = 512;
typedef float knn_f2 __attribute__((ext_vector_type(2)));
__device__ void role_knn(const Ctx& c, const foho_image& im, const Stage2Cfg& cfg, int b, int blk, unsigned char* lds) {
    const int wv = wave_id(), lane = lane_id(), tid = threadIdx.x;
    const int nqb = cfg.nC / cfg.knn_chunks;
    const int oc = blk / nqb, qb = blk - oc * nqb;
    float* s_x = reinterpret_cast<float*>(lds);
    float* s_y = s_x + KNN_ST;
    float* s_z = s_y + KNN_ST;
    unsigned long long* s_best = reinterpret_cast<unsigned long long*>(lds + KNN_ST * 12);
    const int ob = im.v_off + im.Vh, j0 = oc * KNN_CH;
    const bool work = qb * KNN_Q < im.Vh && j0 < im.Vo;
    const int slot = qb * KNN_Q + lane;
    const bool live = work && slot < im.Vh;
    if (!work) return;
    int i = slot;
    if (live && cfg.hand_order_valid) {
        i = slot + c.hand_order[(size_t)b * c.d.Vh_max + slot];
        i = ((unsigned)i < (unsigned)im.Vh) ? i : slot;
    }
    float px, py, pz;
    const int gi_q = im.v_off + min(i, im.Vh - 1);
    {
        px = c.world[3 * gi_q];
        py = c.world[3 * gi_q + 1];
        pz = c.world[3 * gi_q + 2];
    }
    float ub;
    {
        int pj = c.knn_idx[gi_q];
        pj = ((unsigned)pj < (unsigned)im.Vo) ? pj : 0;
        const size_t gp = (size_t)(im.v_off + im.Vh + pj);
        const float dx = px - c.world[3 * gp], dy = py - c.world[3 * gp + 1], dz = pz - c.world[3 * gp + 2];
        ub = live ? dx * dx + dy * dy + dz * dz : -INFINITY;
    }
    const float4* vb4 = reinterpret_cast<const float4*>(c.vbox + ((size_t)b * VERT_BLOCKS_MAX * 4 + (size_t)(j0 / 64)) * 8);
    constexpr int NST = KNN_CH / KNN_ST, PER = KNN_ST / 256;
    float cv[NST][PER][3];
#pragma unroll
    for (int st = 0; st < NST; st++)
#pragma unroll
        for (int u = 0; u < PER; u++) {
            const int j = j0 + st * KNN_ST + u * 256 + tid;
            cv[st][u][0] = cv[st][u][1] = cv[st][u][2] = INFINITY;
            if (j < im.Vo) {
                cv[st][u][0] = c.world[3 * (size_t)(ob + j)];
                cv[st][u][1] = c.world[3 * (size_t)(ob + j) + 1];
                cv[st][u][2] = c.world[3 * (size_t)(ob + j) + 2];
            }
        }
    float bv = INFINITY;
    int bi = 0x7fffffff;
    const knn_f2 qx = {px, px}, qy = {py, py}, qz = {pz, pz};
#pragma unroll
    for (int st = 0; st < NST; st++) {
        if (st) __syncthreads();
#pragma unroll
        for (int u = 0; u < PER; u++) {
            s_x[u * 256 + tid] = cv[st][u][0];
            s_y[u * 256 + tid] = cv[st][u][1];
            s_z[u * 256 + tid] = cv[st][u][2];
        }
        __syncthreads();
        float sv = bv;
        int bg = -1;
        const int w0 = wv * (KNN_ST / 4);
#pragma unroll
        for (int run = 0; run < KNN_ST / 4 / 64; run++) {
        const int e0 = w0 + run * 64;
        {
            const int ru = __builtin_amdgcn_readfirstlane((st * KNN_ST + e0) / 64);
            const float4 blo = vb4[2 * ru], bhi = vb4[2 * ru + 1];
            const float ex = fmaxf(fmaxf(blo.x - px, px - bhi.x), 0.0f), ey = fmaxf(fmaxf(blo.y - py, py - bhi.y), 0.0f),
                        ez = fmaxf(fmaxf(blo.z - pz, pz - bhi.z), 0.0f);
            const float lb = (ex * ex + ey * ey + ez * ez) * 0.99999f;
            if (__builtin_amdgcn_ballot_w64(!(lb > fminf(ub, sv))) == 0ull) continue;
        }
#pragma unroll 2
        for (int e = e0; e < e0 + 64; e += KNN_GRP) {
            float d[KNN_GRP];
#pragma unroll
            for (int h = 0; h < KNN_GRP; h += 4) {
                const float4 ox = *reinterpret_cast<const float4*>(&s_x[e + h]);
                const float4 oy = *reinterpret_cast<const float4*>(&s_y[e + h]);
                const float4 oz = *reinterpret_cast<const float4*>(&s_z[e + h]);
                const knn_f2 dxa = qx - knn_f2{ox.x, ox.y}, dxb = qx - knn_f2{ox.z, ox.w};
                const knn_f2 dya = qy - knn_f2{oy.x, oy.y}, dyb = qy - knn_f2{oy.z, oy.w};
                const knn_f2 dza = qz - knn_f2{oz.x, oz.y}, dzb = qz - knn_f2{oz.z, oz.w};
                const knn_f2 da = dxa * dxa + dya * dya + dza * dza;
                const knn_f2 db = dxb * dxb + dyb * dyb + dzb * dzb;
                d[h] = da.x;
                d[h + 1] = da.y;
                d[h + 2] = db.x;
                d[h + 3] = db.y;
            }
            float gm = fminf(fminf(d[0], d[1]), d[2]);
#pragma unroll
            for (int h = 3; h + 1 < KNN_GRP; h += 2) gm = fminf(fminf(gm, d[h]), d[h + 1]);
            gm = fminf(gm, d[KNN_GRP - 1]);
            if (gm < sv) {
                sv = gm;
                bg = e;
            }
        }
        }
        if (bg >= 0) {
            bv = sv;
            for (int h = KNN_GRP - 1; h >= 0; h--) {
                const float dx = px - s_x[bg + h], dy = py - s_y[bg + h], dz = pz - s_z[bg + h];
                const float d = dx * dx + dy * dy + dz * dz;
                if (d == bv) bi = j0 + st * KNN_ST + bg + h;
            }
        }
    }
    s_best[wv * 64 + lane] = ((unsigned long long)__float_as_uint(bv) << 32) | (unsigned)bi;
    __syncthreads();
    if (live && wv == 0) {
        unsigned long long k = s_best[lane];
        for (int w = 1; w < 4; w++) k = min(k, s_best[w * 64 + lane]);
        const float kb = __uint_as_float((unsigned)(k >> 32));
        if ((unsigned)(k & 0xffffffffull) != 0x7fffffffu && !(kb > ub)) atomicMax(&c.knn_inv[(size_t)b * c.d.Vh_max + i], ~k);
    }
}

__device__ void knn_decode(const Ctx& c, const foho_image& im, float w_contact, float contact_margin, int b, int blk) {
    const int h = blk * 256 + threadIdx.x;
    if (h >= im.Vh || im.Vo <= 0) return;
    const int ob = im.v_off + im.Vh;
    const unsigned long long k = ~c.knn_inv[(size_t)b * c.d.Vh_max + h];
    const float bv = __uint_as_float((unsigned)(k >> 32));
    const int bi = (int)(unsigned)(k & 0xffffffffull);
    const int gi = im.v_off + h;
    c.knn_idx[gi] = bi;
    c.knn_d2[gi] = bv;
    const float a = bv - contact_margin;
    if (a >= 0.0f && w_contact != 0.0f) {
        const int gj = ob + bi;
        const float g = w_contact / (float)im.Vh;
        const float dx = c.world[3 * gi] - c.world[3 * gj], dy = c.world[3 * gi + 1] - c.world[3 * gj + 1],
                    dz = c.world[3 * gi + 2] - c.world[3 * gj + 2];
        atomicAdd(&c.g_world[3 * gj], -2.0f * dx * g);
        atomicAdd(&c.g_world[3 * gj + 1], -2.0f * dy * g);
        atomicAdd(&c.g_world[3 * gj + 2], -2.0f * dz * g);
    }
}
__global__ __launch_bounds__(256) void k_knn_decode(Ctx c, float w_contact, float contact_margin) {
    knn_decode(c, c.img[blockIdx.y], w_contact, contact_margin, blockIdx.y, blockIdx.x);
}

__constant__ int c_tips[5] = {744, 320, 443, 554, 671};
__constant__ int c_kp_order[21] = {0, 13, 14, 15, 16, 1, 2, 3, 17, 4, 5, 6, 18, 10, 11, 12, 19, 7, 8, 9, 20};

__device__ void role_kps(const Ctx& c, const foho_image& im, int b, int blk) {
    const int slot = blk * 4 + wave_id(), lane = lane_id();
    if (slot >= 21) return;
    const int src = c_kp_order[slot];
    float acc[3] = {0.f, 0.f, 0.f};
    if (src < 16) {
        const float* Jr = c.J + (size_t)src * im.jcols;
        for (int v = lane; v < im.jcols; v += 64) {
            const float w = Jr[v];
            const int gv = im.v_off + v;
            acc[0] += w * c.world[3 * gv];
            acc[1] += w * c.world[3 * gv + 1];
            acc[2] += w * c.world[3 * gv + 2];
        }
        for (int k = 0; k < 3; k++) acc[k] = wave_sum(acc[k]);
    } else if (lane == 0) {
        const int gv = im.v_off + c_tips[src - 16];
        for (int k = 0; k < 3; k++) acc[k] = c.world[3 * gv + k];
    }
    if (lane == 0)
        for (int k = 0; k < 3; k++) c.kp3d[((size_t)b * 21 + slot) * 3 + k] = acc[k];
}

__device__ void role_obj_local(const Ctx& c, const foho_image& im, const Stage2Cfg& cfg, int b, int blk, float* red) {
    const int i = blk * 256 + threadIdx.x;
    float v[2] = {0.f, 0.f};
    if (i < im.Vo) {
        const int gv = im.v_off + im.Vh + i;
        const float x = c.world[3 * gv], y = c.world[3 * gv + 1], z = c.world[3 * gv + 2];
        float gx = 0.f, gy = 0.f, gz = 0.f;
        for (int e = c.nbr_off[gv]; e < c.nbr_off[gv + 1]; e++) {
            const int j = c.nbr_idx[e];
            const float dx = x - c.world[3 * j], dy = y - c.world[3 * j + 1], dz = z - c.world[3 * j + 2];
            if (j > gv) v[0] += dx * dx + dy * dy + dz * dz;
            gx += dx;
            gy += dy;
            gz += dz;
        }
        v[1] = x * x + y * y + z * z;
        const float ke = (im.n_edges > 0) ? cfg.w_edge * 2.0f / (float)im.n_edges : 0.0f;
        const float kv = cfg.w_verts * 2.0f / (3.0f * (float)im.Vo);
        c.g_direct[3 * gv] = ke * gx + kv * x;
        c.g_direct[3 * gv + 1] = ke * gy + kv * y;
        c.g_direct[3 * gv + 2] = ke * gz + kv * z;
    }
    block_sum<2>(v, red);
    if (threadIdx.x == 0) {
        float* vp = c.vert_part + ((size_t)b * VERT_BLOCKS_MAX + blk) * 8;
        vp[2] = v[0];
        vp[3] = v[1];
        if (cfg.acc) {
            atomicAdd(&cfg.acc[(size_t)b * SIM_ACC + 34], v[0]);
            atomicAdd(&cfg.acc[(size_t)b * SIM_ACC + 35], v[1]);
        }
    }
}

__device__ void fill_grid_table(const Ctx& c, const float* s_box, float* tab, int nthr) {
    const int res = c.d.grid_res, G1 = res + 1;
    const bool pow2 = (res & (res - 1)) == 0;
    const double inv = 1.0 / (double)res;
    for (int t = threadIdx.x; t < 3 * G1; t += nthr) {
        const int a = (t >= G1) + (t >= 2 * G1), i = t - a * G1;
        const float lo = fminf(s_box[a], s_box[6 + a]);
        const float hi = fmaxf(s_box[3 + a], s_box[9 + a]);
        float v;
        if (i == res) {
            v = hi;
        } else {
            const double ext = (double)hi - (double)lo;
            const double step = pow2 ? ext * inv : ext / (double)res;
            v = (float)((double)i * step + (double)lo);
        }
        tab[t] = v;
    }
}
```

### followmyhold_amd/csrc/k_xform.inc

```

struct XformCfg {
    int nbh, nbo, nz;
    int world_space_input;
    uint4* zero_ptr;
    size_t zero_n16;
    int deferred;
    FinalCfg fin;
};
__global__ __launch_bounds__(256) void k_xform(Ctx c, XformCfg cfg) {
    KSPAN(0);
    __shared__ float s_r[6][4];
    __shared__ float s_newp[16];
    __shared__ float s_fred[36 * 16];
    if ((int)blockIdx.x >= cfg.nbh + cfg.nbo) {
        const size_t nblk = (size_t)cfg.nz * gridDim.y;
        const size_t zb = (size_t)(blockIdx.x - cfg.nbh - cfg.nbo) * gridDim.y + blockIdx.y;
        const uint4 z = {0u, 0u, 0u, 0u};
        for (size_t i = zb * 256 + threadIdx.x; i < cfg.zero_n16; i += nblk * 256) cfg.zero_ptr[i] = z;
        return;
    }
    const int b = blockIdx.y;
    const foho_image im = c.img[b];
    const int mesh = ((int)blockIdx.x < cfg.nbh) ? 0 : 1;
    const int blk = mesh ? (blockIdx.x - cfg.nbh) : blockIdx.x;
    const int n = mesh ? im.Vo : im.Vh;
    if (blk * 256 >= n) return;
    const int base = im.v_off + (mesh ? im.Vh : 0);
    const int i = blk * 256 + threadIdx.x;
    float cen[3];
    mesh_center(c.mesh_info[b * 2 + mesh], cen);
    const float* p = c.params + b * 16 + mesh * 8;
    float v[3] = {0.f, 0.f, 0.f};
    if (i < n) load_moge(c, im, mesh, base + i, v);
    if (cfg.deferred) {
        float* nx = c.state_next + (size_t)b * STATE_NEXT;
        const bool first = blockIdx.x == 0;
        if (first && b == 0) DBG(95);
        FinalPre pre;
        final_prefetch(c, cfg.fin, b, pre);
        if (c.pending[b]) {
            const FinalOut out{nx, nx + 16, nx + 32, reinterpret_cast<int*>(nx) + 48, reinterpret_cast<int*>(nx) + 49, first, s_newp};
            final_role(c, cfg.fin, b, pre, s_fred, out);
        } else {
            if (threadIdx.x < 16) {
                const float pv = c.params[b * 16 + threadIdx.x];
                s_newp[threadIdx.x] = pv;
                if (first) {
                    nx[threadIdx.x] = pv;
                    nx[16 + threadIdx.x] = c.adam_m[b * 16 + threadIdx.x];
                    nx[32 + threadIdx.x] = c.adam_v[b * 16 + threadIdx.x];
                }
            }
            if (first && threadIdx.x == 0) {
                reinterpret_cast<int*>(nx)[48] = c.adam_t[b];
                reinterpret_cast<int*>(nx)[49] = c.flags[b];
            }
        }
        __syncthreads();
        if (first && b == 0) DBG(96);
        p = s_newp + mesh * 8;
    }
    const float s = p[0], tx = p[1], ty = p[2], tz = p[3];
    float Rm[9];
    quat_to_mat(p + 4, Rm);
    float lo[3] = {INFINITY, INFINITY, INFINITY}, hi[3] = {-INFINITY, -INFINITY, -INFINITY};
    if (i < n) {
        const float u0 = s * (v[0] - cen[0]), u1 = s * (v[1] - cen[1]), u2 = s * (v[2] - cen[2]);
        float wx = ((u0 * Rm[0] + u1 * Rm[1]) + u2 * Rm[2] + cen[0]) + tx;
        float wy = ((u0 * Rm[3] + u1 * Rm[4]) + u2 * Rm[5] + cen[1]) + ty;
        float wz = ((u0 * Rm[6] + u1 * Rm[7]) + u2 * Rm[8] + cen[2]) + tz;
        if (cfg.world_space_input) {
            wx = v[0];
            wy = v[1];
            wz = v[2];
        }
        const int gi = base + i;
        c.world[3 * gi] = wx;
        c.world[3 * gi + 1] = wy;
        c.world[3 * gi + 2] = wz;
        const float* Rc = im.cam_R;
        const float vx = ((wx * Rc[0] + wy * Rc[3]) + wz * Rc[6]) + im.cam_T[0];
        const float vy = ((wx * Rc[1] + wy * Rc[4]) + wz * Rc[7]) + im.cam_T[1];
        const float vz = ((wx * Rc[2] + wy * Rc[5]) + wz * Rc[8]) + im.cam_T[2];
        c.ndc[3 * gi] = (im.k00 * vx) / vz;
        c.ndc[3 * gi + 1] = (im.k11 * vy) / vz;
        c.ndc[3 * gi + 2] = vz;
        lo[0] = hi[0] = wx;
        lo[1] = hi[1] = wy;
        lo[2] = hi[2] = wz;
    }
    float* wbox = c.vbox + (((size_t)b * VERT_BLOCKS_MAX + blk) * 4 + wave_id()) * 8;
    for (int a = 0; a < 3; a++) {
        const float x = wave_min(lo[a]), y = wave_max(hi[a]);
        if (lane_id() == 0) {
            s_r[a][wave_id()] = x;
            s_r[3 + a][wave_id()] = y;
            if (mesh) {
                wbox[a] = x;
                wbox[4 + a] = y;
            }
        }
    }
    __syncthreads();
    if (threadIdx.x < 3) {
        const int a = threadIdx.x;
        float* row = c.xf_part + (((size_t)b * 2 + mesh) * VERT_BLOCKS_MAX + blk) * 8;
        row[a] = fminf(fminf(s_r[a][0], s_r[a][1]), fminf(s_r[a][2], s_r[a][3]));
        row[3 + a] = fmaxf(fmaxf(s_r[3 + a][0], s_r[3 + a][1]), fmaxf(s_r[3 + a][2], s_r[3 + a][3]));
    }
}
```

Before: 16150 guidance-steps/s.

## Fuse vertex transform into stage2 kernel and double-buffer zeroed scratch

In deferred mode the separate k_xform launch is removed. Every stage2 role block now runs the deferred optimizer prologue, builds the per-mesh transform in shared memory, and recomputes world or NDC positions on the fly from the raw vertices instead of reading buffers written by a previous kernel. Part of the zeroed scratch (frac/seg counts, rstats, parity, knn_inv) is double-buffered by parity so that k_final and the fused kernel can clear the other half ahead of time. This saves a launch and a global round-trip but adds redundant transform work in every role block, a heavier per-block prologue, and a lower occupancy hint (waves_per_eu 4).

Result: no change. 16110 guidance-steps/s (median of 2 runs) (-0.2%).

```diff
diff --git a/followmyhold_amd/csrc/foho_step.hip b/followmyhold_amd/csrc/foho_step.hip
--- a/followmyhold_amd/csrc/foho_step.hip
+++ b/followmyhold_amd/csrc/foho_step.hip
@@ -112,7 +112,8 @@
     size_t knn_idx, knn_d2, kp3d, g_kp3d, vert_part, sim_part, xf_part, g_special, parity, int_count, final_ticket, knn_inv, loss_acc, vbox, hand_order;
     size_t tile_static, image_static, act_list, act_count;
     int btiles_x, nbtiles;
-    size_t zero_begin, zero_end;
+    size_t zero_begin, zero_mid, zero_end;
+    size_t fz_half[2];
 };
 
 static inline size_t al(size_t x) { return (x + 255) & ~(size_t)255; }
@@ -162,19 +163,20 @@
         w.nseg = nRh + nRo;
     }
     w.seg_count = take(R * B * (size_t)w.nseg * 4);
+    w.rstats = take(R * B * sizeof(RStats));
+    w.parity = take(B * 2 * (size_t)G1 * G1 * 16);
+    w.knn_inv = take(B * (size_t)std::max(d.Vh_max, 1) * 8);
+    w.zero_mid = o;
     w.kfix_count = take(R * B * 4);
     w.hit_count = take(R * B * 4);
     w.bwd_count = take(R * B * 4);
-    w.rstats = take(R * B * sizeof(RStats));
     w.rslot = take(R * B * NSLOT * sizeof(RSlot));
     w.g_world = take(V3);
     w.g_ndc = take(V3);
     w.g_nrm = take(V3);
-    w.parity = take(B * 2 * (size_t)G1 * G1 * 16);
     w.int_count = take(B * 4);
     w.final_ticket = take(B * 4);
     w.loss_acc = take(R * B * LOSS_SLOTS * NPART * 8);
-    w.knn_inv = take(B * (size_t)std::max(d.Vh_max, 1) * 8);
     w.zero_end = o;
     w.clean_begin = o;
     w.zkey = take(R * B * P * 8);
@@ -185,6 +187,8 @@
     w.tile_clean = take(R * B * (size_t)w.nbtiles);
     w.sim_acc = take(2 * B * (size_t)SIM_ACC * 4);
     w.pending = take(B * 4);
+    w.fz_half[0] = take(w.zero_mid - w.zero_begin);
+    w.fz_half[1] = take(w.zero_mid - w.zero_begin);
     w.clean_end = o;
     w.mesh_info = take(B * 2 * sizeof(MeshInfo));
     w.xf_part = take(B * 2 * VERT_BLOCKS_MAX * 8 * 4);
diff --git a/followmyhold_amd/csrc/host.inc b/followmyhold_amd/csrc/host.inc
--- a/followmyhold_amd/csrc/host.inc
+++ b/followmyhold_amd/csrc/host.inc
@@ -255,6 +255,16 @@
     float* acc_prev = deferred ? c.sim_acc + (size_t)(parity ^ 1) * d.B * SIM_ACC : nullptr;
     fc.acc = acc_prev;
     s2.acc = acc_cur;
+    bool fused = deferred && !cfg->world_space_input;
+    if (const char* e = getenv("FOHO_NO_FUSED_XFORM")) fused = fused && strcmp(e, "1") != 0;
+    if (fused) {
+        char* h = (char*)desc->workspace + w.fz_half[parity];
+        c.frac_count = (unsigned*)(h + (w.frac_count - w.zero_begin));
+        c.seg_count = (unsigned*)(h + (w.seg_count - w.zero_begin));
+        c.rstats = (RStats*)(h + (w.rstats - w.zero_begin));
+        c.parity = (unsigned long long*)(h + (w.parity - w.zero_begin));
+        c.knn_inv = (unsigned long long*)(h + (w.knn_inv - w.zero_begin));
+    }
     if (stage_mask & FOHO_STAGE_VERTEX) {
         XformCfg xc{};
         xc.deferred = fc.deferred;
@@ -265,10 +275,22 @@
         xc.zero_ptr = (uint4*)((char*)desc->workspace + w.zero_begin);
         xc.zero_n16 = (w.zero_end - w.zero_begin) / 16;
         xc.nz = (int)std::max<size_t>(1, std::min<size_t>(cdiv((int)std::min<size_t>(xc.zero_n16, 1u << 30), 256 * 4 * d.B), 2048));
-        hipLaunchKernelGGL(k_xform, dim3(nbh + nbo + xc.nz, d.B), dim3(256), 0, stream, c, xc);
-        CHECK_LAUNCH("k_xform");
-        hipLaunchKernelGGL(k_stage2, dim3(s2.nC + s2.nRh + s2.nRo + s2.nI + s2.nA + s2.nD + s2.nE, d.B), dim3(256), 0, stream, c, s2);
-        CHECK_LAUNCH("k_stage2");
+        if (fused) {
+            const int nroles = s2.nC + s2.nRh + s2.nRo + s2.nI + s2.nA + s2.nD + s2.nE;
+            xc.nbh = nroles;
+            xc.nbo = 0;
+            xc.zero_ptr = (uint4*)((char*)desc->workspace + w.zero_mid);
+            xc.zero_n16 = (w.zero_end - w.zero_mid) / 16;
+            xc.zero2_ptr = (uint4*)((char*)desc->workspace + w.fz_half[parity ^ 1]);
+            xc.zero2_n16 = (w.zero_mid - w.zero_begin) / 16;
+            hipLaunchKernelGGL(k_stage2f, dim3(nroles + xc.nz, d.B), dim3(256), 0, stream, c, s2, xc);
+            CHECK_LAUNCH("k_stage2");
+        } else {
+            hipLaunchKernelGGL(k_xform, dim3(nbh + nbo + xc.nz, d.B), dim3(256), 0, stream, c, xc);
+            CHECK_LAUNCH("k_xform");
+            hipLaunchKernelGGL(k_stage2, dim3(s2.nC + s2.nRh + s2.nRo + s2.nI + s2.nA + s2.nD + s2.nE, d.B), dim3(256), 0, stream, c, s2);
+            CHECK_LAUNCH("k_stage2");
+        }
         if (!(stage_mask & FOHO_STAGE_RASTER) && d.Vh_max > 0 && plan.knn_on) {
             hipLaunchKernelGGL(k_knn_decode, dim3(cdiv(d.Vh_max, 256), d.B), dim3(256), 0, stream, c, cfg->w_contact, cfg->contact_margin);
             CHECK_LAUNCH("k_knn_decode");
@@ -368,7 +390,7 @@
         else hipLaunchKernelGGL(k_vert_bwd<2 * VB>, dim3(nvh + nvo, d.B), dim3(256), 0, stream, c, vc);
         CHECK_LAUNCH("k_vert_bwd");
     } else if (stage_mask & FOHO_STAGE_FINAL) {
-        hipLaunchKernelGGL(k_final, dim3(d.B), dim3(256), 0, stream, c, fc);
+        hipLaunchKernelGGL(k_final, dim3(d.B), dim3(256), 0, stream, c, fc, (uint4*)nullptr, (size_t)0);
         CHECK_LAUNCH("k_final");
     }
     return FOHO_OK;
@@ -396,7 +418,9 @@
     fc.deferred = 1;
     fc.acc = c.sim_acc + (size_t)((cfg->deferred_update - 1) & 1) * d.B * SIM_ACC;
     hipStream_t stream = (hipStream_t)stream_;
-    hipLaunchKernelGGL(k_final, dim3(d.B), dim3(256), 0, stream, c, fc);
+    const size_t zn16 = (w.fz_half[1] + (w.zero_mid - w.zero_begin) - w.fz_half[0]) / 16;
+    const int nzb = (int)std::max<size_t>(1, std::min<size_t>((zn16 + 256 * 4 - 1) / (256 * 4), 256));
+    hipLaunchKernelGGL(k_final, dim3(d.B + nzb), dim3(256), 0, stream, c, fc, (uint4*)((char*)desc->workspace + w.fz_half[0]), zn16);
     CHECK_LAUNCH("k_final");
     return FOHO_OK;
 }
diff --git a/followmyhold_amd/csrc/k_final.inc b/followmyhold_amd/csrc/k_final.inc
--- a/followmyhold_amd/csrc/k_final.inc
+++ b/followmyhold_amd/csrc/k_final.inc
@@ -304,8 +304,14 @@
     return FinalOut{c.params + b * 16, c.adam_m + b * 16, c.adam_v + b * 16, c.adam_t + b, c.flags + b, true, nullptr};
 }
 
-__global__ __launch_bounds__(256) void k_final(Ctx c, FinalCfg cfg) {
+__global__ __launch_bounds__(256) void k_final(Ctx c, FinalCfg cfg, uint4* zp, size_t zn16) {
     __shared__ float red[36 * 16];
+    if ((int)blockIdx.x >= c.d.B) {
+        const size_t nblk = gridDim.x - c.d.B;
+        const uint4 z = {0u, 0u, 0u, 0u};
+        for (size_t i = ((size_t)blockIdx.x - c.d.B) * 256 + threadIdx.x; i < zn16; i += nblk * 256) zp[i] = z;
+        return;
+    }
     const int b = blockIdx.x;
     if (cfg.deferred && !c.pending[b]) return;
     FinalPre pre;
diff --git a/followmyhold_amd/csrc/k_inside.inc b/followmyhold_amd/csrc/k_inside.inc
--- a/followmyhold_amd/csrc/k_inside.inc
+++ b/followmyhold_amd/csrc/k_inside.inc
@@ -82,7 +82,7 @@
     unsigned off[IF + 1];
 };
 
-__device__ void inside_faces_role(const Ctx& c, const Stage2Cfg& cfg, int b, int blk, InsideLds& L) {
+__device__ void inside_faces_role(const Ctx& c, const Stage2Cfg& cfg, int b, int blk, InsideLds& L, const float* xf = nullptr) {
     const foho_image im = c.img[b];
     const int res = c.d.grid_res, G1 = res + 1;
     const int tid = threadIdx.x;
@@ -100,10 +100,10 @@
     if (live) {
         const int f = im.f_off + lf;
         for (int k = 0; k < 3; k++) id[k] = c.faces[3 * f + k];
-        for (int k = 0; k < 3; k++)
-            for (int q = 0; q < 3; q++) P[3 * k + q] = c.world[3 * id[k] + q];
+        for (int k = 0; k < 3; k++) ld_world(c, im, xf, id[k], &P[3 * k]);
     }
-    world_boxes(c, im, b, L.box);
+    if (xf) world_boxes_xf(c, im, xf, L.box, L.tab, lean);
+    else world_boxes(c, im, b, L.box);
     fill_grid_table(c, L.box, L.tab, lean);
     __syncthreads();
     if (direct) {
diff --git a/followmyhold_amd/csrc/k_raster.inc b/followmyhold_amd/csrc/k_raster.inc
--- a/followmyhold_amd/csrc/k_raster.inc
+++ b/followmyhold_amd/csrc/k_raster.inc
@@ -60,7 +60,7 @@
     return !((face_set == FOHO_FACES_HAND && !is_hand) || (face_set == FOHO_FACES_OBJ && is_hand));
 }
 
-__device__ void role_raster(const Ctx& c, const foho_image& im, const Stage2Cfg& cfg, int b, int blk, RasterLds& rl) {
+__device__ void role_raster(const Ctx& c, const foho_image& im, const Stage2Cfg& cfg, int b, int blk, RasterLds& rl, const float* xf = nullptr) {
     const int tid = threadIdx.x;
     const int H = c.d.H, W = c.d.W;
     const bool objblk = blk >= cfg.nRh;
@@ -93,9 +93,15 @@
             for (int k = 0; k < 3; k++) vi[k] = c.faces[3 * f + k];
             if (dbgr) DBGW(dslot + 6);
             for (int k = 0; k < 3; k++) {
-                fv[3 * k] = c.ndc[3 * vi[k]];
-                fv[3 * k + 1] = c.ndc[3 * vi[k] + 1];
-                fv[3 * k + 2] = c.ndc[3 * vi[k] + 2];
+                if (xf) {
+                    float w[3];
+                    xf_world(c, im, xf, objblk ? 1 : 0, vi[k], w);
+                    project_vertex(im, w, &fv[3 * k]);
+                } else {
+                    fv[3 * k] = c.ndc[3 * vi[k]];
+                    fv[3 * k + 1] = c.ndc[3 * vi[k] + 1];
+                    fv[3 * k + 2] = c.ndc[3 * vi[k] + 2];
+                }
             }
             if (dbgr) DBGW(dslot + 7);
             for (int k = 0; k < 9; k++) {
@@ -300,39 +306,48 @@
     if (dbgr && tid == 0) DBG_VALUE(dslot + 8, T);
 }
 
+constexpr size_t KNN_LDS = (size_t)KNN_ST * 12 + 256 * 8 + (KNN_CH / 64) * 32;
+constexpr size_t RI_LDS = sizeof(RasterLds) > sizeof(InsideLds) ? sizeof(RasterLds) : sizeof(InsideLds);
+constexpr size_t STAGE2_LDS = RI_LDS > KNN_LDS ? RI_LDS : KNN_LDS;
+
+__device__ __forceinline__ int stage2_lean(const Stage2Cfg& cfg) {
+    int k = (int)blockIdx.x - cfg.nC, lean_role = 256;
+    if (k >= 0) {
+        if (k < cfg.nRh) lean_role = cfg.lean_h;
+        else if (k < cfg.nRh + cfg.nRo) lean_role = cfg.lean_o;
+        else if (k - cfg.nRh - cfg.nRo < cfg.nI) lean_role = (k - cfg.nRh - cfg.nRo < cfg.nIh || cfg.if_o != IFO) ? cfg.lean_i : 256;
+    }
+    return lean_role;
+}
+
+__device__ __forceinline__ void stage2_roles(const Ctx& c, const Stage2Cfg& cfg, const foho_image& im, int b, unsigned char* s_raw, float* red,
+                                             const float* xf) {
+    RasterLds& rl = *reinterpret_cast<RasterLds*>(s_raw);
+    int blk = blockIdx.x;
+    if (blk < cfg.nC) return role_knn(c, im, cfg, b, xcd_order(blk, cfg.nC), s_raw, xf);
+    blk -= cfg.nC;
+    if (blk < cfg.nRh + cfg.nRo)
+        return role_raster(c, im, cfg, b, blk < cfg.nRh ? blk : cfg.nRh + xcd_order(blk - cfg.nRh, cfg.nRo), rl, xf);
+    blk -= cfg.nRh + cfg.nRo;
+    if (blk < cfg.nI)
+        return inside_faces_role(c, cfg, b, blk < cfg.nIh ? blk : cfg.nIh + xcd_order(blk - cfg.nIh, cfg.nI - cfg.nIh),
+                                 *reinterpret_cast<InsideLds*>(s_raw), xf);
+    blk -= cfg.nI;
+    if (blk < cfg.nA) return role_normals(c, im, cfg, xcd_order(blk, cfg.nA), xf);
+    blk -= cfg.nA;
+    if (blk < cfg.nD) return role_kps(c, im, b, blk, xf);
+    blk -= cfg.nD;
+    if (blk < cfg.nE) return role_obj_local(c, im, cfg, b, xcd_order(blk, cfg.nE), red, xf);
+}
+
 __global__ __launch_bounds__(256) __attribute__((amdgpu_waves_per_eu(7, 7))) void k_stage2(Ctx c, Stage2Cfg cfg) {
     KSPAN(1);
     __shared__ float red[32];
-    constexpr size_t knn_lds = (size_t)KNN_ST * 12 + 256 * 8;
-    constexpr size_t ri_lds = sizeof(RasterLds) > sizeof(InsideLds) ? sizeof(RasterLds) : sizeof(InsideLds);
-    __shared__ __align__(16) unsigned char s_raw[ri_lds > knn_lds ? ri_lds : knn_lds];
-    RasterLds& rl = *reinterpret_cast<RasterLds*>(s_raw);
-    {
-        int k = (int)blockIdx.x - cfg.nC, lean_role = 256;
-        if (k >= 0) {
-            if (k < cfg.nRh) lean_role = cfg.lean_h;
-            else if (k < cfg.nRh + cfg.nRo) lean_role = cfg.lean_o;
-            else if (k - cfg.nRh - cfg.nRo < cfg.nI) lean_role = (k - cfg.nRh - cfg.nRo < cfg.nIh || cfg.if_o != IFO) ? cfg.lean_i : 256;
-        }
-        if ((int)threadIdx.x >= lean_role) return;
-    }
+    __shared__ __align__(16) unsigned char s_raw[STAGE2_LDS];
+    if ((int)threadIdx.x >= stage2_lean(cfg)) return;
     const int b = blockIdx.y;
     const foho_image im = c.img[b];
-    int blk = blockIdx.x;
-    if (blk < cfg.nC) return role_knn(c, im, cfg, b, xcd_order(blk, cfg.nC), s_raw);
-    blk -= cfg.nC;
-    if (blk < cfg.nRh + cfg.nRo)
-        return role_raster(c, im, cfg, b, blk < cfg.nRh ? blk : cfg.nRh + xcd_order(blk - cfg.nRh, cfg.nRo), rl);
-    blk -= cfg.nRh + cfg.nRo;
-    if (blk < cfg.nI)
-        return inside_faces_role(c, cfg, b, blk < cfg.nIh ? blk : cfg.nIh + xcd_order(blk - cfg.nIh, cfg.nI - cfg.nIh),
-                                 *reinterpret_cast<InsideLds*>(s_raw));
-    blk -= cfg.nI;
-    if (blk < cfg.nA) return role_normals(c, im, cfg, xcd_order(blk, cfg.nA));
-    blk -= cfg.nA;
-    if (blk < cfg.nD) return role_kps(c, im, b, blk);
-    blk -= cfg.nD;
-    if (blk < cfg.nE) return role_obj_local(c, im, cfg, b, xcd_order(blk, cfg.nE), red);
+    stage2_roles(c, cfg, im, b, s_raw, red, nullptr);
 }
 
 __device__ __forceinline__ void kbuffer_fix(const Ctx& c, const RasterCfg& cfg, const foho_image& im, int rbi, int f0r, int f1r, int px,
diff --git a/followmyhold_amd/csrc/k_vertex.inc b/followmyhold_amd/csrc/k_vertex.inc
--- a/followmyhold_amd/csrc/k_vertex.inc
+++ b/followmyhold_amd/csrc/k_vertex.inc
@@ -10,6 +10,40 @@
         v[0] = ((x * M[0] + y * M[1]) + z * M[2]) + M[3];
         v[1] = ((x * M[4] + y * M[5]) + z * M[6]) + M[7];
         v[2] = ((x * M[8] + y * M[9]) + z * M[10]) + M[11];
+    }
+}
+
+constexpr int XF_N = 16;
+__device__ __forceinline__ void xform_vertex(const float* X, const float* v, float* w) {
+    const float s = X[0], tx = X[1], ty = X[2], tz = X[3];
+    const float* Rm = X + 4;
+    const float* cen = X + 13;
+    const float u0 = s * (v[0] - cen[0]), u1 = s * (v[1] - cen[1]), u2 = s * (v[2] - cen[2]);
+    w[0] = ((u0 * Rm[0] + u1 * Rm[1]) + u2 * Rm[2] + cen[0]) + tx;
+    w[1] = ((u0 * Rm[3] + u1 * Rm[4]) + u2 * Rm[5] + cen[1]) + ty;
+    w[2] = ((u0 * Rm[6] + u1 * Rm[7]) + u2 * Rm[8] + cen[2]) + tz;
+}
+__device__ __forceinline__ void project_vertex(const foho_image& im, const float* w, float* o) {
+    const float* Rc = im.cam_R;
+    const float vx = ((w[0] * Rc[0] + w[1] * Rc[3]) + w[2] * Rc[6]) + im.cam_T[0];
+    const float vy = ((w[0] * Rc[1] + w[1] * Rc[4]) + w[2] * Rc[7]) + im.cam_T[1];
+    const float vz = ((w[0] * Rc[2] + w[1] * Rc[5]) + w[2] * Rc[8]) + im.cam_T[2];
+    o[0] = (im.k00 * vx) / vz;
+    o[1] = (im.k11 * vy) / vz;
+    o[2] = vz;
+}
+__device__ __forceinline__ void xf_world(const Ctx& c, const foho_image& im, const float* xf, int mesh, int gi, float* w) {
+    float v[3];
+    load_moge(c, im, mesh, gi, v);
+    xform_vertex(xf + XF_N * mesh, v, w);
+}
+__device__ __forceinline__ void ld_world(const Ctx& c, const foho_image& im, const float* xf, int gi, float* w) {
+    if (xf) {
+        xf_world(c, im, xf, (gi - im.v_off) >= im.Vh ? 1 : 0, gi, w);
+    } else {
+        w[0] = c.world[3 * (size_t)gi];
+        w[1] = c.world[3 * (size_t)gi + 1];
+        w[2] = c.world[3 * (size_t)gi + 2];
     }
 }
 
@@ -92,6 +126,37 @@
     __syncthreads();
 }
 
+__device__ void world_boxes_xf(const Ctx& c, const foho_image& im, const float* xf, float* s_box, float* scr, int nthr) {
+    float v[12];
+    for (int mesh = 0; mesh < 2; mesh++) {
+        for (int a = 0; a < 3; a++) {
+            v[6 * mesh + a] = INFINITY;
+            v[6 * mesh + 3 + a] = -INFINITY;
+        }
+        const int n = mesh ? im.Vo : im.Vh, base = im.v_off + (mesh ? im.Vh : 0);
+        for (int i = threadIdx.x; i < n; i += nthr) {
+            float w[3];
+            xf_world(c, im, xf, mesh, base + i, w);
+            for (int a = 0; a < 3; a++) {
+                v[6 * mesh + a] = fminf(v[6 * mesh + a], w[a]);
+                v[6 * mesh + 3 + a] = fmaxf(v[6 * mesh + 3 + a], w[a]);
+            }
+        }
+    }
+    for (int q = 0; q < 12; q++) {
+        const float x = ((q % 6) < 3) ? wave_min(v[q]) : wave_max(v[q]);
+        if (lane_id() == 0) scr[wave_id() * 12 + q] = x;
+    }
+    __syncthreads();
+    if (threadIdx.x < 12) {
+        const int q = threadIdx.x, nw = nthr / 64;
+        float x = scr[q];
+        for (int w = 1; w < nw; w++) x = ((q % 6) < 3) ? fminf(x, scr[w * 12 + q]) : fmaxf(x, scr[w * 12 + q]);
+        s_box[q] = x;
+    }
+    __syncthreads();
+}
+
 struct Stage2Cfg {
     int nA, nC, nD, nE, nI;
     int lean_h, lean_o, lean_i;
@@ -109,11 +174,20 @@
     float w_edge, w_verts, w_contact, contact_margin;
 };
 
-__device__ void role_normals(const Ctx& c, const foho_image& im, const Stage2Cfg& cfg, int blk) {
+__device__ void role_normals(const Ctx& c, const foho_image& im, const Stage2Cfg& cfg, int blk, const float* xf = nullptr) {
     const int i = blk * 256 + threadIdx.x;
     if (i >= im.Vh + im.Vo) return;
+    const int gv = im.v_off + i;
+    if (xf) {
+        float w[3], o[3];
+        xf_world(c, im, xf, i >= im.Vh ? 1 : 0, gv, w);
+        project_vertex(im, w, o);
+        for (int k = 0; k < 3; k++) {
+            c.world[3 * gv + k] = w[k];
+            c.ndc[3 * gv + k] = o[k];
+        }
+    }
     if (!((i < im.Vh) ? cfg.vn_hand : cfg.vn_obj)) return;
-    const int gv = im.v_off + i;
     float acc[3] = {0.f, 0.f, 0.f};
     const int e0 = c.inc_off[gv], e1 = c.inc_off[gv + 1];
     for (int base = e0; base < e1; base += 8) {
@@ -127,7 +201,7 @@
 #pragma unroll
         for (int u = 0; u < 8; u++)
             for (int k = 0; k < 3; k++)
-                for (int q = 0; q < 3; q++) P[u][3 * k + q] = c.world[3 * vi[u][k] + q];
+                ld_world(c, im, xf, vi[u][k], &P[u][3 * k]);
 #pragma unroll
         for (int u = 0; u < 8; u++) {
             if (base + u >= e1) break;
@@ -195,7 +269,7 @@
 constexpr int KNN_Q = 64, KNN_CH = 1024, KNN_GRP = 8;
 constexpr int KNN_ST = 512;
 typedef float knn_f2 __attribute__((ext_vector_type(2)));
-__device__ void role_knn(const Ctx& c, const foho_image& im, const Stage2Cfg& cfg, int b, int blk, unsigned char* lds) {
+__device__ void role_knn(const Ctx& c, const foho_image& im, const Stage2Cfg& cfg, int b, int blk, unsigned char* lds, const float* xf = nullptr) {
     const int wv = wave_id(), lane = lane_id(), tid = threadIdx.x;
     const int nqb = cfg.nC / cfg.knn_chunks;
     const int oc = blk / nqb, qb = blk - oc * nqb;
@@ -203,6 +277,7 @@
     float* s_y = s_x + KNN_ST;
     float* s_z = s_y + KNN_ST;
     unsigned long long* s_best = reinterpret_cast<unsigned long long*>(lds + KNN_ST * 12);
+    float* s_vb = reinterpret_cast<float*>(lds + KNN_ST * 12 + 256 * 8);
     const int ob = im.v_off + im.Vh, j0 = oc * KNN_CH;
     const bool work = qb * KNN_Q < im.Vh && j0 < im.Vo;
     const int slot = qb * KNN_Q + lane;
@@ -216,16 +291,19 @@
     float px, py, pz;
     const int gi_q = im.v_off + min(i, im.Vh - 1);
     {
-        px = c.world[3 * gi_q];
-        py = c.world[3 * gi_q + 1];
-        pz = c.world[3 * gi_q + 2];
+        float w[3];
+        ld_world(c, im, xf, gi_q, w);
+        px = w[0];
+        py = w[1];
+        pz = w[2];
     }
     float ub;
     {
         int pj = c.knn_idx[gi_q];
         pj = ((unsigned)pj < (unsigned)im.Vo) ? pj : 0;
-        const size_t gp = (size_t)(im.v_off + im.Vh + pj);
-        const float dx = px - c.world[3 * gp], dy = py - c.world[3 * gp + 1], dz = pz - c.world[3 * gp + 2];
+        float w[3];
+        ld_world(c, im, xf, im.v_off + im.Vh + pj, w);
+        const float dx = px - w[0], dy = py - w[1], dz = pz - w[2];
         ub = live ? dx * dx + dy * dy + dz * dz : -INFINITY;
     }
     const float4* vb4 = reinterpret_cast<const float4*>(c.vbox + ((size_t)b * VERT_BLOCKS_MAX * 4 + (size_t)(j0 / 64)) * 8);
@@ -237,10 +315,16 @@
         for (int u = 0; u < PER; u++) {
             const int j = j0 + st * KNN_ST + u * 256 + tid;
             cv[st][u][0] = cv[st][u][1] = cv[st][u][2] = INFINITY;
-            if (j < im.Vo) {
-                cv[st][u][0] = c.world[3 * (size_t)(ob + j)];
-                cv[st][u][1] = c.world[3 * (size_t)(ob + j) + 1];
-                cv[st][u][2] = c.world[3 * (size_t)(ob + j) + 2];
+            if (j < im.Vo) ld_world(c, im, xf, ob + j, cv[st][u]);
+            if (xf) {
+                float* row = s_vb + (st * (KNN_ST / 64) + u * 4 + wv) * 8;
+                for (int a = 0; a < 3; a++) {
+                    const float x = wave_min(cv[st][u][a]), y = wave_max(j < im.Vo ? cv[st][u][a] : -INFINITY);
+                    if (lane == 0) {
+                        row[a] = x;
+                        row[4 + a] = y;
+                    }
+                }
             }
         }
     float bv = INFINITY;
@@ -264,7 +348,14 @@
         const int e0 = w0 + run * 64;
         {
             const int ru = __builtin_amdgcn_readfirstlane((st * KNN_ST + e0) / 64);
-            const float4 blo = vb4[2 * ru], bhi = vb4[2 * ru + 1];
+            float4 blo, bhi;
+            if (xf) {
+                blo = reinterpret_cast<const float4*>(s_vb)[2 * ru];
+                bhi = reinterpret_cast<const float4*>(s_vb)[2 * ru + 1];
+            } else {
+                blo = vb4[2 * ru];
+                bhi = vb4[2 * ru + 1];
+            }
             const float ex = fmaxf(fmaxf(blo.x - px, px - bhi.x), 0.0f), ey = fmaxf(fmaxf(blo.y - py, py - bhi.y), 0.0f),
                         ez = fmaxf(fmaxf(blo.z - pz, pz - bhi.z), 0.0f);
             const float lb = (ex * ex + ey * ey + ez * ez) * 0.99999f;
@@ -345,7 +436,7 @@
 __constant__ int c_tips[5] = {744, 320, 443, 554, 671};
 __constant__ int c_kp_order[21] = {0, 13, 14, 15, 16, 1, 2, 3, 17, 4, 5, 6, 18, 10, 11, 12, 19, 7, 8, 9, 20};
 
-__device__ void role_kps(const Ctx& c, const foho_image& im, int b, int blk) {
+__device__ void role_kps(const Ctx& c, const foho_image& im, int b, int blk, const float* xf = nullptr) {
     const int slot = blk * 4 + wave_id(), lane = lane_id();
     if (slot >= 21) return;
     const int src = c_kp_order[slot];
@@ -355,29 +446,35 @@
         for (int v = lane; v < im.jcols; v += 64) {
             const float w = Jr[v];
             const int gv = im.v_off + v;
-            acc[0] += w * c.world[3 * gv];
-            acc[1] += w * c.world[3 * gv + 1];
-            acc[2] += w * c.world[3 * gv + 2];
+            float p[3];
+            ld_world(c, im, xf, gv, p);
+            acc[0] += w * p[0];
+            acc[1] += w * p[1];
+            acc[2] += w * p[2];
         }
         for (int k = 0; k < 3; k++) acc[k] = wave_sum(acc[k]);
     } else if (lane == 0) {
         const int gv = im.v_off + c_tips[src - 16];
-        for (int k = 0; k < 3; k++) acc[k] = c.world[3 * gv + k];
+        ld_world(c, im, xf, gv, acc);
     }
     if (lane == 0)
         for (int k = 0; k < 3; k++) c.kp3d[((size_t)b * 21 + slot) * 3 + k] = acc[k];
 }
 
-__device__ void role_obj_local(const Ctx& c, const foho_image& im, const Stage2Cfg& cfg, int b, int blk, float* red) {
+__device__ void role_obj_local(const Ctx& c, const foho_image& im, const Stage2Cfg& cfg, int b, int blk, float* red, const float* xf = nullptr) {
     const int i = blk * 256 + threadIdx.x;
     float v[2] = {0.f, 0.f};
     if (i < im.Vo) {
         const int gv = im.v_off + im.Vh + i;
-        const float x = c.world[3 * gv], y = c.world[3 * gv + 1], z = c.world[3 * gv + 2];
+        float p[3];
+        ld_world(c, im, xf, gv, p);
+        const float x = p[0], y = p[1], z = p[2];
         float gx = 0.f, gy = 0.f, gz = 0.f;
         for (int e = c.nbr_off[gv]; e < c.nbr_off[gv + 1]; e++) {
             const int j = c.nbr_idx[e];
-            const float dx = x - c.world[3 * j], dy = y - c.world[3 * j + 1], dz = z - c.world[3 * j + 2];
+            float pj[3];
+            ld_world(c, im, xf, j, pj);
+            const float dx = x - pj[0], dy = y - pj[1], dz = z - pj[2];
             if (j > gv) v[0] += dx * dx + dy * dy + dz * dz;
             gx += dx;
             gy += dy;
diff --git a/followmyhold_amd/csrc/k_xform.inc b/followmyhold_amd/csrc/k_xform.inc
--- a/followmyhold_amd/csrc/k_xform.inc
+++ b/followmyhold_amd/csrc/k_xform.inc
@@ -4,9 +4,38 @@
     int world_space_input;
     uint4* zero_ptr;
     size_t zero_n16;
+    uint4* zero2_ptr;
+    size_t zero2_n16;
     int deferred;
     FinalCfg fin;
 };
+__device__ __forceinline__ void deferred_prologue(const Ctx& c, const FinalCfg& fin, int b, bool first, float* s_newp, float* s_fred) {
+    float* nx = c.state_next + (size_t)b * STATE_NEXT;
+    if (first && b == 0) DBG(95);
+    FinalPre pre;
+    final_prefetch(c, fin, b, pre);
+    if (c.pending[b]) {
+        const FinalOut out{nx, nx + 16, nx + 32, reinterpret_cast<int*>(nx) + 48, reinterpret_cast<int*>(nx) + 49, first, s_newp};
+        final_role(c, fin, b, pre, s_fred, out);
+    } else {
+        if (threadIdx.x < 16) {
+            const float pv = c.params[b * 16 + threadIdx.x];
+            s_newp[threadIdx.x] = pv;
+            if (first) {
+                nx[threadIdx.x] = pv;
+                nx[16 + threadIdx.x] = c.adam_m[b * 16 + threadIdx.x];
+                nx[32 + threadIdx.x] = c.adam_v[b * 16 + threadIdx.x];
+            }
+        }
+        if (first && threadIdx.x == 0) {
+            reinterpret_cast<int*>(nx)[48] = c.adam_t[b];
+            reinterpret_cast<int*>(nx)[49] = c.flags[b];
+        }
+    }
+    __syncthreads();
+    if (first && b == 0) DBG(96);
+}
+
 __global__ __launch_bounds__(256) void k_xform(Ctx c, XformCfg cfg) {
     KSPAN(0);
     __shared__ float s_r[6][4];
@@ -33,58 +62,31 @@
     float v[3] = {0.f, 0.f, 0.f};
     if (i < n) load_moge(c, im, mesh, base + i, v);
     if (cfg.deferred) {
-        float* nx = c.state_next + (size_t)b * STATE_NEXT;
-        const bool first = blockIdx.x == 0;
-        if (first && b == 0) DBG(95);
-        FinalPre pre;
-        final_prefetch(c, cfg.fin, b, pre);
-        if (c.pending[b]) {
-            const FinalOut out{nx, nx + 16, nx + 32, reinterpret_cast<int*>(nx) + 48, reinterpret_cast<int*>(nx) + 49, first, s_newp};
-            final_role(c, cfg.fin, b, pre, s_fred, out);
-        } else {
-            if (threadIdx.x < 16) {
-                const float pv = c.params[b * 16 + threadIdx.x];
-                s_newp[threadIdx.x] = pv;
-                if (first) {
-                    nx[threadIdx.x] = pv;
-                    nx[16 + threadIdx.x] = c.adam_m[b * 16 + threadIdx.x];
-                    nx[32 + threadIdx.x] = c.adam_v[b * 16 + threadIdx.x];
-                }
-            }
-            if (first && threadIdx.x == 0) {
-                reinterpret_cast<int*>(nx)[48] = c.adam_t[b];
-                reinterpret_cast<int*>(nx)[49] = c.flags[b];
-            }
-        }
-        __syncthreads();
-        if (first && b == 0) DBG(96);
+        deferred_prologue(c, cfg.fin, b, blockIdx.x == 0, s_newp, s_fred);
         p = s_newp + mesh * 8;
     }
-    const float s = p[0], tx = p[1], ty = p[2], tz = p[3];
-    float Rm[9];
-    quat_to_mat(p + 4, Rm);
+    float X[XF_N];
+    for (int k = 0; k < 4; k++) X[k] = p[k];
+    quat_to_mat(p + 4, X + 4);
+    for (int k = 0; k < 3; k++) X[13 + k] = cen[k];
     float lo[3] = {INFINITY, INFINITY, INFINITY}, hi[3] = {-INFINITY, -INFINITY, -INFINITY};
     if (i < n) {
-        const float u0 = s * (v[0] - cen[0]), u1 = s * (v[1] - cen[1]), u2 = s * (v[2] - cen[2]);
-        float wx = ((u0 * Rm[0] + u1 * Rm[1]) + u2 * Rm[2] + cen[0]) + tx;
-        float wy = ((u0 * Rm[3] + u1 * Rm[4]) + u2 * Rm[5] + cen[1]) + ty;
-        float wz = ((u0 * Rm[6] + u1 * Rm[7]) + u2 * Rm[8] + cen[2]) + tz;
+        float w[3], o[3];
+        xform_vertex(X, v, w);
         if (cfg.world_space_input) {
-            wx = v[0];
-            wy = v[1];
-            wz = v[2];
+            w[0] = v[0];
+            w[1] = v[1];
+            w[2] = v[2];
         }
+        const float wx = w[0], wy = w[1], wz = w[2];
         const int gi = base + i;
         c.world[3 * gi] = wx;
         c.world[3 * gi + 1] = wy;
         c.world[3 * gi + 2] = wz;
-        const float* Rc = im.cam_R;
-        const float vx = ((wx * Rc[0] + wy * Rc[3]) + wz * Rc[6]) + im.cam_T[0];
-        const float vy = ((wx * Rc[1] + wy * Rc[4]) + wz * Rc[7]) + im.cam_T[1];
-        const float vz = ((wx * Rc[2] + wy * Rc[5]) + wz * Rc[8]) + im.cam_T[2];
-        c.ndc[3 * gi] = (im.k00 * vx) / vz;
-        c.ndc[3 * gi + 1] = (im.k11 * vy) / vz;
-        c.ndc[3 * gi + 2] = vz;
+        project_vertex(im, w, o);
+        c.ndc[3 * gi] = o[0];
+        c.ndc[3 * gi + 1] = o[1];
+        c.ndc[3 * gi + 2] = o[2];
         lo[0] = hi[0] = wx;
         lo[1] = hi[1] = wy;
         lo[2] = hi[2] = wz;
@@ -109,3 +111,39 @@
         row[3 + a] = fmaxf(fmaxf(s_r[3 + a][0], s_r[3 + a][1]), fmaxf(s_r[3 + a][2], s_r[3 + a][3]));
     }
 }
+
+__global__ __launch_bounds__(256) __attribute__((amdgpu_waves_per_eu(4, 4))) void k_stage2f(Ctx c, Stage2Cfg cfg, XformCfg xc) {
+    KSPAN(1);
+    __shared__ float red[32];
+    __shared__ float s_newp[16];
+    __shared__ __align__(16) float s_xf[2 * XF_N];
+    __shared__ __align__(16) unsigned char s_raw[STAGE2_LDS];
+    if ((int)blockIdx.x >= xc.nbh) {
+        const size_t nblk = (size_t)xc.nz * gridDim.y;
+        const size_t zb = (size_t)(blockIdx.x - xc.nbh) * gridDim.y + blockIdx.y;
+        const uint4 z = {0u, 0u, 0u, 0u};
+        for (size_t i = zb * 256 + threadIdx.x; i < xc.zero_n16; i += nblk * 256) xc.zero_ptr[i] = z;
+        for (size_t i = zb * 256 + threadIdx.x; i < xc.zero2_n16; i += nblk * 256) xc.zero2_ptr[i] = z;
+        return;
+    }
+    const int b = blockIdx.y;
+    deferred_prologue(c, xc.fin, b, blockIdx.x == 0, s_newp, reinterpret_cast<float*>(s_raw));
+    if ((int)threadIdx.x >= stage2_lean(cfg)) return;
+    if (threadIdx.x < 2 * XF_N) {
+        const int mesh = threadIdx.x / XF_N, k = threadIdx.x % XF_N;
+        float cen[3], Rm[9];
+        mesh_center(c.mesh_info[b * 2 + mesh], cen);
+        quat_to_mat(s_newp + mesh * 8 + 4, Rm);
+        float x = s_newp[mesh * 8 + (k & 3)];
+#pragma unroll
+        for (int q = 0; q < 9; q++)
+            if (k == 4 + q) x = Rm[q];
+#pragma unroll
+        for (int q = 0; q < 3; q++)
+            if (k == 13 + q) x = cen[q];
+        s_xf[threadIdx.x] = x;
+    }
+    __syncthreads();
+    const foho_image im = c.img[b];
+    stage2_roles(c, cfg, im, b, s_raw, red, s_xf);
+}
```
